# hellozhuo/svnet

Hardware: AMD Instinct MI355X
Metric: point-clouds/sec fwd+bwd, sv_dgcnn_cls B=32 N=1024 k=20 (higher is better)
Workload: dtype f32 (ternary bit-planes in the binarized layers); 1 GPU; sv_dgcnn_cls --binary fwd+loss+bwd, B=32 per GPU, N=1024, k=20; global_batch=32, parallelism=dp1, collective=none (1 rank), rccl_world=1, launch=hipGraph replay, binlinear=i8_mfma (>= 1024 rows) + xnor (head)

## Files before the change

include/svnet_hip.h:

```cpp
#ifndef SVNET_HIP_H
#define SVNET_HIP_H

#include <stddef.h>
#include <stdint.h>

#ifdef __cplusplus
extern "C" {
#endif

#define SVNET_OK 0
#define SVNET_E_ARG (-1)
#define SVNET_E_UNSUPPORTED (-2)
#define SVNET_E_WORKSPACE (-3)
#define SVNET_E_LAUNCH (-4)

#define SVNET_RED_SLICES 16
#define SVNET_SLICED_LEN(L) ((SVNET_RED_SLICES + 1) * (L) + 2)
int svnet_slices_sum_f32(float* buf, int64_t L, void* stream);
int svnet_slices_sum_f64(double* buf, int64_t L, void* stream);

#define SVNET_ABI_VERSION 417
int svnet_version(void);
const char* svnet_last_error(void);

typedef struct svnet_gate_fwd_job {
    const float* gin; const double* gin_f64; float* gin_out; float in_scale; const float* W0; const float* W2;
    int64_t B, Cin, H, Ov; float* h; float* gate;
    const float* rows; int64_t R;
} svnet_gate_fwd_job;
typedef struct svnet_gate_bwd_job {
    const float* dgate; const float* gate; const float* h; const float* gin; float in_scale; const float* W0; const float* W2;
    int64_t B, Cin, H, Ov; float out_scale; float* dgin; float* dW0; float* dW2;
} svnet_gate_bwd_job;

size_t svnet_knn_workspace_bytes(int64_t B, int64_t N, int64_t C);
int svnet_knn_f32(const float* x, int64_t B, int64_t N, int64_t C, int64_t sb, int64_t sn, int64_t sc,
                  int xx_mode, int k, int64_t* idx_out, void* workspace, size_t workspace_bytes, void* stream);
int svnet_knn_sv_f32(const float* s, int64_t Cs, const float* v, int64_t Cv3, int64_t B, int64_t N, int k, int64_t* idx_out,
                     void* workspace, size_t workspace_bytes, void* stream);

int svnet_knn_table_fusable(int64_t B, int64_t N, int64_t C);
int svnet_knn_from_table_f32(const void* workspace, size_t workspace_bytes, int64_t B, int64_t N, int64_t C, int k, int64_t* idx_out,
                             void* stream);
int svnet_edgeblock_apply_knn_f32(const int32_t* n_max, const int32_t* n_min, const float* mv, const float* mvn, const float* coef,
                                  const float* gate, int64_t P, int64_t N, int64_t Os, int64_t Ov, float slope, float* s_out, float* v_out,
                                  float* s_cat, int64_t s_ld, float* v_cat, int64_t v_ld, void* knn_workspace, size_t knn_workspace_bytes,
                                  void* stream);
int svnet_xyzblock_apply_knn_f32(const float* y_max, const float* y_min, const float* mv, const float* mvn, const float* coef,
                                 const float* gate, int64_t P, int64_t N, int64_t Os, int64_t Ov, float slope, float* s_out, float* v_out,
                                 float* s_cat, int64_t s_ld, float* v_cat, int64_t v_ld, void* knn_workspace, size_t knn_workspace_bytes,
                                 void* stream);

int svnet_edge_xyz_f32(const float* x, const int64_t* idx, int64_t B, int64_t N, int64_t k, int64_t m, int mode,
                       float* out, void* stream);

int svnet_edge_diffcat_fwd_f32(const float* table, const int64_t* idx, int idx_is_global, int64_t B, int64_t N,
                               int64_t k, int64_t G, int64_t F, float* out, void* stream);
int svnet_edge_diffcat_bwd_f32(const float* d_out, const int64_t* idx, int idx_is_global, int64_t B, int64_t N,
                               int64_t k, int64_t G, int64_t F, float* d_table, void* stream);

typedef struct svnet_gemm_desc {
    int64_t M, N, K;
    const float* A; int64_t a_rs, a_cs;
    const float* a_scale;
    const uint64_t* a_sign; const uint64_t* a_nz;
    const float* B; int64_t b_rs, b_cs;
    int b_exact;
    float* C; int64_t ldc, c_cs;
    float alpha;
    const float* col_scale;
    const float* bias;
    const uint64_t* mask;
    float* col_sum;
    int split_k;
    int accumulate;
    uint32_t tern_tile_mask;
    void* workspace;
    size_t workspace_bytes;
} svnet_gemm_desc;
size_t svnet_gemm_workspace_bytes(int64_t N, int64_t K);
int svnet_gemm_f32(const svnet_gemm_desc* desc, void* stream);

int svnet_binweight_prepare_f32(const float* W, const float* scale, int64_t O, int64_t K, uint64_t* w_sign,
                                uint64_t* w_nz, float* w_b, float* w_eff, void* stream);
int svnet_binlinear_fwd_f32(const float* x, int64_t ldx, const float* beta, const uint64_t* w_sign,
                            const uint64_t* w_nz, const float* scale, const float* bias, int64_t M, int64_t K,
                            int64_t O, float* y, uint64_t* x_sign, uint64_t* x_nz, uint64_t* x_ste, void* stream);
size_t svnet_binweight_i8_bytes(int64_t O, int64_t K);
int svnet_binweight_pack_i8(const float* W, int64_t O, int64_t K, int8_t* w_i8, void* stream);
int svnet_binlinear_i8_fwd_f32(const float* x, int64_t ldx, const float* beta, const int8_t* w_i8, const float* scale,
                               const float* bias, int64_t M, int64_t K, int64_t O, float* y, uint64_t* x_sign, uint64_t* x_nz,
                               uint64_t* x_ste, double* col_sums, void* stream);
int svnet_binlinear_i8_cloud_fwd_f32(const float* x, int64_t ldx, const float* beta, const int8_t* w_i8, const float* scale,
                                     const float* bias, int64_t M, int64_t K, int64_t O, float* y, uint64_t* x_sign, uint64_t* x_nz,
                                     uint64_t* x_ste, double* col_sums, const float* cloud_n, int64_t rows_per_cloud, void* stream);
int svnet_binweight_grad_f32(const float* GX, const float* W, const float* scale, int64_t O, int64_t K,
                             float* dW, float* dscale, int accumulate, int gx_sliced, float* sum_buf, int64_t sum_len, void* stream);

typedef struct svnet_edgeblock_desc {
    int64_t B, N, k;
    int Cs, Cv, Os, Ov;
    const float* s; const float* v; const int64_t* idx;
    const float* zz; const float* ut;
    const uint64_t* w_sign; const uint64_t* w_nz; const float* beta_perm;
    int32_t* n_max; int32_t* n_min; uint8_t* slot_max; uint8_t* slot_min;
    float* mv; float* mvn;
    int64_t* stat_n; double* stat_v; double* gate_sum;
    int16_t* n16; uint64_t* planes;
    const uint32_t* w_dense;
} svnet_edgeblock_desc;
int svnet_edgeblock_prepare_f32(const float* W, const float* beta, int64_t Os, int64_t Cs, int64_t Cv, uint64_t* w_sign,
                                uint64_t* w_nz, float* beta_perm , void* stream);
int svnet_edgeblock_prepare_vec_f32(const float* W2, const float* scale2, const float* Wz, const float* scalez, int64_t Ov,
                                    int64_t Cv, float* wv, float* scv, void* stream);
int svnet_edgeblock_fwd_f32(const svnet_edgeblock_desc* desc, void* stream);
int svnet_edgeblock_coeffs_f32(const int64_t* stat_n, const double* stat_v, int64_t E, int64_t Os, int64_t Ov,
                               const float* scale1, const float* gamma1, const float* beta1, float* running_mean1,
                               float* running_var1, const float* gamma2, const float* beta2, float* running_mean2,
                               float* running_var2, int training, float eps, float momentum, float* coef,
                               int64_t* num_batches_tracked1, int64_t* num_batches_tracked2 ,
                               const svnet_gate_fwd_job* gate_job , void* stream);
int svnet_edgeblock_apply_f32(const int32_t* n_max, const int32_t* n_min, const float* mv, const float* mvn,
                              const float* coef, const float* gate, int64_t P, int64_t N, int64_t Os, int64_t Ov,
                              float slope, float* s_out, float* v_out, float* s_cat, int64_t s_ld, float* v_cat, int64_t v_ld,
                              void* stream);

typedef struct svnet_block_tail_desc {
    const void* stat1; const double* stat_v; int64_t E, Os, Ov;
    const float* scale1;
    const float* gamma1; const float* beta1; float* running_mean1; float* running_var1;
    const float* gamma2; const float* beta2; float* running_mean2; float* running_var2;
    int training; float eps, momentum;
    float* coef; int64_t* num_batches_tracked1; int64_t* num_batches_tracked2;
    svnet_gate_fwd_job gate;
    const void* hi; const void* lo; const float* mv; const float* mvn;
    int64_t P, N; float slope;
    float* s_out; float* v_out; float* s_cat; int64_t s_ld; float* v_cat; int64_t v_ld;
    void* knn_workspace; size_t knn_workspace_bytes;
} svnet_block_tail_desc;
int svnet_block_tail_supported(int64_t P, int64_t N, int64_t Os, int64_t Ov, int with_knn_table);
int svnet_edgeblock_tail_f32(const svnet_block_tail_desc* desc, void* stream);
int svnet_xyzblock_tail_f32(const svnet_block_tail_desc* desc, void* stream);

#define SVNET_DBETA_SLICES 64
typedef struct svnet_edgeblock_bwd_desc {
    int64_t B, N, k;
    int Cs, Cv, Os, Ov;
    const float* v; const int64_t* idx; const float* zz; const float* ut;
    const int16_t* n16; const uint64_t* planes;
    const uint16_t* w1bt;
    const float* scale1;
    const uint8_t* slot_max; const uint8_t* slot_min;
    const float* coef;
    const float* gate;
    const float* gy;
    const float* bcoef;
    const float* gv;
    const float* gconst;
    float* dn_out; uint32_t* x_sign32; uint32_t* x_nz32;
    float* msg;
    float* ub_tab; float* ge_tab;
    float* ds_acc; float* dv_acc; float* dvc; float* dzc; float* dbeta_perm;
    int64_t* debug;
    int parts;
} svnet_edgeblock_bwd_desc;
int svnet_edgeblock_wbt_bf16(const uint64_t* w_sign, const uint64_t* w_nz, int64_t Os, int64_t Cs, int64_t Cv, uint16_t* wbt,
                             uint32_t* w_dense, void* stream);
int svnet_edgeblock_bwd_prelude_f32(const float* gs, const float* gv, const int32_t* n_max, const int32_t* n_min,
                                    const float* mv, const float* mvn, const float* coef, const float* scale1,
                                    const float* gate, int64_t P, int64_t N, int64_t Os, int64_t Ov, float slope,
                                    float* gy, float* red, float* redv, float* dgate,
                                    const float* gs2, int64_t gs2_ld, const float* gv2, int64_t gv2_ld, float* gv_sum, void* stream);
int svnet_edgeblock_bwd_coeffs_f32(const float* red, const float* redv, const float* coef, const float* gamma1,
                                   const float* gamma2, int64_t E, int64_t Os, int64_t Ov, int training, const float* scale1,
                                   float* bcoef, float* dgamma1, float* dbeta1, float* dgamma2, float* dbeta2,
                                   const svnet_gate_bwd_job* gate_job , void* stream);
int svnet_edgeblock_bwd_f32(const svnet_edgeblock_bwd_desc* desc, void* stream);
int svnet_knn_reverse_i32(const int64_t* idx, int64_t B, int64_t N, int64_t k, int32_t* rev_range, int32_t* rev_edge,
                          int32_t* rev_src, int64_t chunk, int32_t* ovf_items, int32_t* ovf_count, void* stream);
int64_t svnet_edgeblock_msg_stride(int64_t Cs, int64_t Cv, int64_t Ov);
int svnet_edgeblock_bwd_gather_f32(const float* msg, const int32_t* rev_range, const int32_t* rev_edge, const int32_t* rev_src,
                                   const float* ut, const float* ub_tab, const float* ge_tab, const float* coef, const float* bcoef,
                                   int64_t Os, const float* dvc, const float* dzc, int64_t P ,
                                   int64_t N , int64_t Cs, int64_t Cv,
                                   int64_t Ov, float* acat,
                                   int64_t acat_ld ,
                                   float* ds_acc, float* dv_acc, const float* dbeta_perm, float* dbeta1,
                                   int64_t chunk, const int32_t* ovf_items, const int32_t* ovf_count , void* stream);
int svnet_edgeblock_bwd_params_f32(const float* GXp, const float* GXc, const float* W1, const float* scale1, const float* W2,
                                   const float* scale2, const float* Wz, const float* scalez, int64_t Os, int64_t Ov,
                                   int64_t Cs, int64_t Cv, float* dW1, float* dscale1, float* dW2, float* dscale2, float* dWz,
                                   float* dscalez, void* stream);

typedef struct svnet_xyzblock_desc {
    int64_t B, N, k;
    int Os, Ov;
    const float* x; const int64_t* idx;
    const float* w0; const float* wz; const float* w1; const float* w2;
    float* y_max; float* y_min; uint8_t* slot_max; uint8_t* slot_min;
    float* mv; float* mvn;
    double* stat_y; double* stat_v; double* gate_sum;
    int64_t nc;
} svnet_xyzblock_desc;
int svnet_xyzblock_fwd_f32(const svnet_xyzblock_desc* desc, void* stream);
int svnet_xyzblock_coeffs_f32(const double* stat_y, const double* stat_v, int64_t E, int64_t Os, int64_t Ov,
                              const float* gamma1, const float* beta1, float* running_mean1, float* running_var1,
                              const float* gamma2, const float* beta2, float* running_mean2, float* running_var2,
                              int training, float eps, float momentum, float* coef, int64_t* num_batches_tracked1,
                              int64_t* num_batches_tracked2, const svnet_gate_fwd_job* gate_job , void* stream);
int svnet_xyzblock_apply_f32(const float* y_max, const float* y_min, const float* mv, const float* mvn, const float* coef,
                             const float* gate, int64_t P, int64_t N, int64_t Os, int64_t Ov, float slope, float* s_out,
                             float* v_out, float* s_cat, int64_t s_ld, float* v_cat, int64_t v_ld ,
                             void* stream);
int svnet_xyzblock_bwd_prelude_f32(const float* gs, const float* gv, const float* y_max, const float* y_min, const float* mv,
                                   const float* mvn, const float* coef, const float* gate, int64_t P, int64_t N, int64_t Os,
                                   int64_t Ov, float slope, float* gy, float* red, float* redv, float* dgate, const float* gs2,
                                   int64_t gs2_ld, const float* gv2, int64_t gv2_ld, float* gv_sum ,
                                   void* stream);
typedef struct svnet_xyzblock_bwd_desc {
    int64_t B, N, k;
    int Os, Ov;
    const float* x; const int64_t* idx;
    const float* w0; const float* wz; const float* w1; const float* w2;
    const uint8_t* slot_max; const uint8_t* slot_min;
    const float* coef; const float* bcoef; const float* gate; const float* gy; const float* gv; const float* gconst;
    float* gw;
    int64_t nc;
} svnet_xyzblock_bwd_desc;
int svnet_xyzblock_bwd_f32(const svnet_xyzblock_bwd_desc* desc, void* stream);

int svnet_edgeblock_wgrad_f32(const int16_t* n16, const uint8_t* slot_max, const uint8_t* slot_min, const float* gy,
                              const float* chc, const uint64_t* x_sign, const uint64_t* x_nz, int64_t E, int64_t k, int64_t Os,
                              float* GX, uint32_t q_tile_mask, void* stream);

int svnet_v2s_fwd_f32(const float* v, const float* w_eff, int64_t M, int64_t C, int64_t J, float* s, float* z_out,
                      void* stream);
int svnet_v2s_bwd_f32(const float* v, const float* w_eff, const float* ds, const float* dz_in, int64_t M, int64_t C,
                      int64_t J, float* dv, float* GX, void* stream);
int svnet_v2s_cat_fwd_f32(const float* v, const float* w_eff, const float* pre, int64_t pre_cols, int64_t M, int64_t C, int64_t J,
                          float* out, int64_t out_ld, void* stream);
int svnet_v2s_cat_sum_supported(int64_t M, int64_t C, int64_t pre_cols, int64_t rows_per_cloud);
int svnet_v2s_cat_sum_fwd_f32(const float* v, const float* w_eff, const float* pre, int64_t pre_cols, int64_t M, int64_t C, int64_t multi,
                              float* out, int64_t out_ld, double* pre_sum, int64_t rows_per_cloud, void* stream);
int svnet_v2s_bwd_ld_f32(const float* v, const float* w_eff, const float* ds, int64_t ds_ld, const float* dz_in, int64_t M, int64_t C,
                         int64_t J, float* dv, float* GX, void* stream);
int svnet_vproject_fwd_f32(const float* v, const float* z, int64_t M, int64_t C, int64_t J, float* s, void* stream);
int svnet_vproject_bwd_f32(const float* v, const float* z, const float* ds, int64_t M, int64_t C, int64_t J, float* dv,
                           float* dz, void* stream);

int svnet_colstats_f64(const float* x, int64_t M, int64_t C, int kind, double* sums, void* stream);
int svnet_vlinear_stats_f32(const float* v, int64_t P, int64_t K, const float* w_b, const float* col_scale, int64_t O, float* y,
                            double* sums, void* stream);
int svnet_bn_finalize_f32(double* sums, int64_t M, int64_t C, float eps, float momentum, float* mean,
                          float* invstd, float* running_mean, float* running_var, int64_t* num_batches_tracked,
                          void* stream);
int svnet_bn_eval_stats_f32(const float* running_mean, const float* running_var, int64_t C, float eps, float* mean,
                            float* invstd, void* stream);
int svnet_bn_act_fwd_f32(const float* x, const float* mean, const float* invstd, const float* gamma,
                         const float* beta, int64_t M, int64_t C, int act, float slope, float* y, void* stream);
int svnet_bn_act_bwd_reduce_f32(const float* g, const float* x, const float* mean, const float* invstd,
                                const float* gamma, const float* beta, int64_t M, int64_t C, int act, float slope,
                                float* red, void* stream);
int svnet_bn_act_bwd_apply_f32(const float* g, const float* x, const float* mean, const float* invstd,
                               const float* gamma, const float* beta, float* red, int64_t M, int64_t C, int act,
                               float slope, int train_stats, float* dx, void* stream);

int svnet_vbn_fwd_f32(const float* v, const float* mean, const float* invstd, const float* gamma, const float* beta,
                      const float* gate, int64_t rows_per_batch, int64_t M, int64_t C, float* out, void* stream);
int svnet_vbn_fwd_stats_f32(const float* v, const double* sums, float eps, float momentum, float* mean, float* invstd,
                            float* running_mean, float* running_var, int64_t* num_batches_tracked, const float* gamma,
                            const float* beta, const float* gate, int64_t rows_per_batch, int64_t M, int64_t C, float* out,
                            void* stream);
int svnet_vbn_bwd_reduce_f32(const float* g, const float* v, const float* mean, const float* invstd,
                             const float* gamma, const float* beta, const float* gate, int64_t rows_per_batch,
                             int64_t M, int64_t C, float* red, float* dgate, void* stream);
int svnet_vbn_bwd_apply_f32(const float* g, const float* v, const float* mean, const float* invstd,
                            const float* gamma, const float* beta, const float* gate, float* red,
                            int64_t rows_per_batch, int64_t M, int64_t C, int train_stats, float* dv, void* stream);

size_t svnet_pool_workspace_bytes(int64_t outer, int64_t R, int64_t inner, int mode);
int svnet_pool_fwd_f32(const float* x, int64_t outer, int64_t R, int64_t inner, int mode, float* out, int64_t out_ld,
                       int32_t* argmax, void* workspace, size_t workspace_bytes, void* stream);
int svnet_pool_maxmean_fwd_f32(const float* x, int64_t outer, int64_t R, int64_t inner, float* out_max, float* out_mean,
                               int64_t out_ld, int32_t* argmax, void* workspace, size_t workspace_bytes, void* stream);
int svnet_bn_pool_fwd_f32(const float* y, const float* mean, const float* invstd, const float* gamma, const float* beta,
                          int64_t outer, int64_t R, int64_t inner, int act, float slope, float* out_max, float* out_mean,
                          int64_t out_ld, int32_t* argmax, void* workspace, size_t workspace_bytes,
                          int workspace_zeroed ,
                          void* stream);
int svnet_bn_pool_bwd_f32(const float* gmax, const float* gmean, int64_t g_ld, const int32_t* argmax, const float* y,
                          const float* mean, const float* invstd, const float* gamma, const float* beta, int64_t outer, int64_t R,
                          int64_t inner, int act, float slope, int train_stats, float* red, float* dy, void* stream);
int svnet_pool_bwd_f32(const float* g, const int32_t* argmax, int64_t outer, int64_t R, int64_t inner, int mode,
                       float* dx, void* stream);
size_t svnet_vtail_workspace_bytes(int64_t B, int64_t N, int64_t C);
int svnet_vtail_fwd_f32(const float* v, const double* sums, float eps, float momentum, float* mean, float* invstd,
                        float* running_mean, float* running_var, long long* nbt, const float* gamma, const float* beta,
                        const float* gate, const float* w_eff, int64_t B, int64_t N, int64_t C, float* out_max, float* out_mean,
                        int64_t out_ld, int32_t* argmax, void* workspace, size_t workspace_bytes,
                        int workspace_zeroed , void* stream);
int svnet_vtail_bwd_f32(const float* v, const float* mean, const float* invstd, const float* gamma, const float* beta,
                        const float* gate, const float* w_eff, const float* gmax, const float* gmean, int64_t g_ld,
                        const int32_t* argmax, int64_t B, int64_t N, int64_t C, float* red, float* dgate, float* GX, float* g5,
                        void* stream);
int svnet_vtail_bwd_apply_f32(const float* v, const float* mean, const float* invstd, const float* gamma, const float* beta,
                              const float* gate, const float* w_eff, const float* gmax, const float* gmean, int64_t g_ld,
                              const int32_t* argmax, int64_t B, int64_t N, int64_t C, float* red, int train_stats, float* dv, void* stream);
int svnet_pool_mean_bwd_add_f32(const float* gmean, const float* add, int64_t add_ld, int64_t outer, int64_t R, int64_t inner,
                                float* dx, void* stream);
int svnet_pool_maxmean_bwd_f32(const float* gmax, const float* gmean, int64_t g_ld, const int32_t* argmax, int64_t outer, int64_t R,
                               int64_t inner, float* dx, void* stream);

int svnet_act_fwd_f32(const float* x, int64_t n, int kind, float* y, void* stream);
int svnet_act_bwd_f32(const float* g, const float* y, int64_t n, int kind, float* dx, void* stream);

int svnet_gate_mlp_fwd_f32(const float* gin, const double* gin_f64, float* gin_out, float in_scale, const float* W0,
                           const float* W2, int64_t B, int64_t Cin, int64_t H, int64_t Ov, float* h, float* gate,
                           const float* rows , int64_t R , void* stream);
int svnet_gate_mlp_bwd_f32(const float* dgate, const float* gate, const float* h, const float* gin, float in_scale,
                           const float* W0, const float* W2, int64_t B, int64_t Cin, int64_t H, int64_t Ov, float out_scale,
                           float* dgin, float* dW0, float* dW2, void* stream);

typedef struct svnet_binhead_desc {
    int64_t M, K, O;
    const float* W;
    const uint64_t* w_sign;
    const uint64_t* w_nz;
    int64_t wld;
    const float* w_b;
    const float* scale;
    const float* gamma;
    const float* bn_beta;
    float* running_mean;
    float* running_var;
    long long* nbt;
    int training;
    float eps, momentum;
    int act;
    float slope;
    const uint64_t* x_sign;
    const uint64_t* x_nz;
    const uint64_t* x_ste;
    const uint64_t* xc_sign;
    const uint64_t* xc_nz;
    float* y;
    float* mean;
    float* invstd;
    float* out;
    const float* g;
    float* dnT;
    float* dW;
    float* dscale;
    float* dgamma;
    float* dbn_beta;
    float* dx;
    float* dbeta_in;
} svnet_binhead_desc;
int svnet_binhead_pack_f32(const float* x, const float* beta, int64_t M, int64_t K, uint64_t* x_sign, uint64_t* x_nz,
                           uint64_t* x_ste, uint64_t* xc_sign, uint64_t* xc_nz, uint64_t* xc_ste, void* stream);
int svnet_binhead_fwd_f32(const svnet_binhead_desc* d, void* stream);
int svnet_binhead_bwd_f32(const svnet_binhead_desc* d, void* stream);
int svnet_fplinear_small_bwd_f32(const float* g, const float* x, const float* W, int64_t M, int64_t K, int64_t O, float* dx,
                                 float* dW, float* db, void* stream);

int svnet_smooth_ce_f32(const float* logits, const int64_t* target, int64_t R, int64_t C, float eps, float* loss,
                        float* dlogits, float* workspace, int64_t workspace_floats, void* stream);

int svnet_adam_step_f32(float* p, const float* g, float* m, float* v, int64_t n, float lr, float beta1, float beta2, float eps,
                        float weight_decay, int64_t step, void* stream);
int svnet_sgd_step_f32(float* p, const float* g, float* buf, int64_t n, float lr, float momentum, float weight_decay,
                       int first_step, void* stream);
int svnet_adam_step_dev_f32(float* p, const float* g, float* m, float* v, int64_t n, const float* hyper, void* stream);
int svnet_sgd_step_dev_f32(float* p, const float* g, float* buf, int64_t n, const float* hyper, void* stream);

int svnet_stamp_u64(uint64_t* slot, void* stream);

#ifdef __cplusplus
}
#endif
#endif
```

svnet_amd/_lib.py:

```python
import ctypes
import os
import subprocess

_HERE = os.path.dirname(os.path.abspath(__file__))
LIB_PATH = os.environ.get("SVNET_DIAG_LIB") or os.path.join(_HERE, "libsvnet_hip.so")
_lib = None
ABI_VERSION = 417

c_p = ctypes.c_void_p
c_i64 = ctypes.c_int64
c_int = ctypes.c_int
c_f = ctypes.c_float
c_sz = ctypes.c_size_t


class GemmDesc(ctypes.Structure):
    _fields_ = [
        ("M", c_i64), ("N", c_i64), ("K", c_i64),
        ("A", c_p), ("a_rs", c_i64), ("a_cs", c_i64),
        ("a_scale", c_p),
        ("a_sign", c_p), ("a_nz", c_p),
        ("B", c_p), ("b_rs", c_i64), ("b_cs", c_i64),
        ("b_exact", c_int),
        ("C", c_p), ("ldc", c_i64), ("c_cs", c_i64),
        ("alpha", c_f),
        ("col_scale", c_p),
        ("bias", c_p),
        ("mask", c_p),
        ("col_sum", c_p),
        ("split_k", c_int),
        ("accumulate", c_int),
        ("tern_tile_mask", ctypes.c_uint32),
        ("workspace", c_p),
        ("workspace_bytes", ctypes.c_size_t),
    ]


class GateFwdJob(ctypes.Structure):
    _fields_ = [("gin", c_p), ("gin_f64", c_p), ("gin_out", c_p), ("in_scale", c_f), ("W0", c_p), ("W2", c_p),
                ("B", c_i64), ("Cin", c_i64), ("H", c_i64), ("Ov", c_i64), ("h", c_p), ("gate", c_p), ("rows", c_p), ("R", c_i64)]


class BlockTailDesc(ctypes.Structure):
    _fields_ = [("stat1", c_p), ("stat_v", c_p), ("E", c_i64), ("Os", c_i64), ("Ov", c_i64), ("scale1", c_p),
                ("gamma1", c_p), ("beta1", c_p), ("running_mean1", c_p), ("running_var1", c_p),
                ("gamma2", c_p), ("beta2", c_p), ("running_mean2", c_p), ("running_var2", c_p),
                ("training", c_int), ("eps", c_f), ("momentum", c_f),
                ("coef", c_p), ("num_batches_tracked1", c_p), ("num_batches_tracked2", c_p),
                ("gate", GateFwdJob),
                ("hi", c_p), ("lo", c_p), ("mv", c_p), ("mvn", c_p), ("P", c_i64), ("N", c_i64), ("slope", c_f),
                ("s_out", c_p), ("v_out", c_p), ("s_cat", c_p), ("s_ld", c_i64), ("v_cat", c_p), ("v_ld", c_i64),
                ("knn_workspace", c_p), ("knn_workspace_bytes", c_sz)]


class GateBwdJob(ctypes.Structure):
    _fields_ = [("dgate", c_p), ("gate", c_p), ("h", c_p), ("gin", c_p), ("in_scale", c_f), ("W0", c_p), ("W2", c_p),
                ("B", c_i64), ("Cin", c_i64), ("H", c_i64), ("Ov", c_i64), ("out_scale", c_f), ("dgin", c_p), ("dW0", c_p), ("dW2", c_p)]


class EdgeBlockDesc(ctypes.Structure):
    _fields_ = [
        ("B", c_i64), ("N", c_i64), ("k", c_i64),
        ("Cs", c_int), ("Cv", c_int), ("Os", c_int), ("Ov", c_int),
        ("s", c_p), ("v", c_p), ("idx", c_p),
        ("zz", c_p), ("ut", c_p),
        ("w_sign", c_p), ("w_nz", c_p), ("beta_perm", c_p),
        ("n_max", c_p), ("n_min", c_p), ("slot_max", c_p), ("slot_min", c_p),
        ("mv", c_p), ("mvn", c_p),
        ("stat_n", c_p), ("stat_v", c_p), ("gate_sum", c_p),
        ("n16", c_p), ("planes", c_p),
        ("w_dense", c_p),
    ]


class EdgeBlockBwdDesc(ctypes.Structure):
    _fields_ = [
        ("B", c_i64), ("N", c_i64), ("k", c_i64),
        ("Cs", c_int), ("Cv", c_int), ("Os", c_int), ("Ov", c_int),
        ("v", c_p), ("idx", c_p), ("zz", c_p), ("ut", c_p),
        ("n16", c_p), ("planes", c_p),
        ("w1bt", c_p),
        ("scale1", c_p),
        ("slot_max", c_p), ("slot_min", c_p),
        ("coef", c_p), ("gate", c_p), ("gy", c_p), ("bcoef", c_p), ("gv", c_p), ("gconst", c_p),
        ("dn_out", c_p), ("x_sign32", c_p), ("x_nz32", c_p),
        ("msg", c_p),
        ("ub_tab", c_p), ("ge_tab", c_p),
        ("ds_acc", c_p), ("dv_acc", c_p), ("dvc", c_p), ("dzc", c_p), ("dbeta_perm", c_p),
        ("debug", c_p),
        ("parts", c_int),
    ]


class XyzBlockDesc(ctypes.Structure):
    _fields_ = [
        ("B", c_i64), ("N", c_i64), ("k", c_i64),
        ("Os", c_int), ("Ov", c_int),
        ("x", c_p), ("idx", c_p),
        ("w0", c_p), ("wz", c_p), ("w1", c_p), ("w2", c_p),
        ("y_max", c_p), ("y_min", c_p), ("slot_max", c_p), ("slot_min", c_p),
        ("mv", c_p), ("mvn", c_p),
        ("stat_y", c_p), ("stat_v", c_p), ("gate_sum", c_p),
        ("nc", c_i64),
    ]


class XyzBlockBwdDesc(ctypes.Structure):
    _fields_ = [
        ("B", c_i64), ("N", c_i64), ("k", c_i64),
        ("Os", c_int), ("Ov", c_int),
        ("x", c_p), ("idx", c_p),
        ("w0", c_p), ("wz", c_p), ("w1", c_p), ("w2", c_p),
        ("slot_max", c_p), ("slot_min", c_p),
        ("coef", c_p), ("bcoef", c_p), ("gate", c_p), ("gy", c_p), ("gv", c_p), ("gconst", c_p),
        ("gw", c_p),
        ("nc", c_i64),
    ]


class BinHeadDesc(ctypes.Structure):
    _fields_ = [
        ("M", c_i64), ("K", c_i64), ("O", c_i64),
        ("W", c_p), ("w_sign", c_p), ("w_nz", c_p), ("wld", c_i64), ("w_b", c_p),
        ("scale", c_p), ("gamma", c_p), ("bn_beta", c_p),
        ("running_mean", c_p), ("running_var", c_p), ("nbt", c_p),
        ("training", c_int), ("eps", c_f), ("momentum", c_f), ("act", c_int), ("slope", c_f),
        ("x_sign", c_p), ("x_nz", c_p), ("x_ste", c_p), ("xc_sign", c_p), ("xc_nz", c_p),
        ("y", c_p), ("mean", c_p), ("invstd", c_p), ("out", c_p),
        ("g", c_p), ("dnT", c_p), ("dW", c_p), ("dscale", c_p), ("dgamma", c_p), ("dbn_beta", c_p),
        ("dx", c_p), ("dbeta_in", c_p),
    ]


SIGNATURES = {
    "svnet_version": (c_int, []),
    "svnet_stamp_u64": (c_int, [c_p, c_p]),
    "svnet_slices_sum_f32": (c_int, [c_p, c_i64, c_p]),
    "svnet_slices_sum_f64": (c_int, [c_p, c_i64, c_p]),
    "svnet_last_error": (ctypes.c_char_p, []),
    "svnet_knn_workspace_bytes": (c_sz, [c_i64, c_i64, c_i64]),
    "svnet_knn_f32": (c_int, [c_p, c_i64, c_i64, c_i64, c_i64, c_i64, c_i64, c_int, c_int, c_p, c_p, c_sz, c_p]),
    "svnet_knn_sv_f32": (c_int, [c_p, c_i64, c_p, c_i64, c_i64, c_i64, c_int, c_p, c_p, c_sz, c_p]),
    "svnet_knn_table_fusable": (c_int, [c_i64, c_i64, c_i64]),
    "svnet_block_tail_supported": (c_int, [c_i64, c_i64, c_i64, c_i64, c_int]),
    "svnet_edgeblock_tail_f32": (c_int, [c_p, c_p]),
    "svnet_xyzblock_tail_f32": (c_int, [c_p, c_p]),
    "svnet_knn_from_table_f32": (c_int, [c_p, c_sz, c_i64, c_i64, c_i64, c_int, c_p, c_p]),
    "svnet_edge_xyz_f32": (c_int, [c_p, c_p, c_i64, c_i64, c_i64, c_i64, c_int, c_p, c_p]),
    "svnet_edge_diffcat_fwd_f32": (c_int, [c_p, c_p, c_int, c_i64, c_i64, c_i64, c_i64, c_i64, c_p, c_p]),
    "svnet_edge_diffcat_bwd_f32": (c_int, [c_p, c_p, c_int, c_i64, c_i64, c_i64, c_i64, c_i64, c_p, c_p]),
    "svnet_gemm_workspace_bytes": (ctypes.c_size_t, [c_i64, c_i64]),
    "svnet_gemm_f32": (c_int, [ctypes.POINTER(GemmDesc), c_p]),
    "svnet_binweight_prepare_f32": (c_int, [c_p, c_p, c_i64, c_i64, c_p, c_p, c_p, c_p, c_p]),
    "svnet_binlinear_fwd_f32": (c_int, [c_p, c_i64, c_p, c_p, c_p, c_p, c_p, c_i64, c_i64, c_i64, c_p, c_p, c_p, c_p, c_p]),
    "svnet_binweight_grad_f32": (c_int, [c_p, c_p, c_p, c_i64, c_i64, c_p, c_p, c_int, c_int, c_p, c_i64, c_p]),
    "svnet_edgeblock_prepare_vec_f32": (c_int, [c_p, c_p, c_p, c_p, c_i64, c_i64, c_p, c_p, c_p]),
    "svnet_knn_reverse_i32": (c_int, [c_p, c_i64, c_i64, c_i64, c_p, c_p, c_p, c_i64, c_p, c_p, c_p]),
    "svnet_edgeblock_msg_stride": (c_i64, [c_i64, c_i64, c_i64]),
    "svnet_edgeblock_bwd_gather_f32": (c_int, [c_p] * 9 + [c_i64] + [c_p, c_p] + [c_i64] * 5 + [c_p, c_i64, c_p, c_p, c_p, c_p, c_i64, c_p, c_p, c_p]),
    "svnet_edgeblock_bwd_params_f32": (c_int, [c_p] * 8 + [c_i64] * 4 + [c_p] * 6 + [c_p]),
    "svnet_edgeblock_prepare_f32": (c_int, [c_p, c_p, c_i64, c_i64, c_i64, c_p, c_p, c_p, c_p]),
    "svnet_edgeblock_fwd_f32": (c_int, [ctypes.POINTER(EdgeBlockDesc), c_p]),
    "svnet_edgeblock_coeffs_f32": (c_int, [c_p, c_p, c_i64, c_i64, c_i64, c_p, c_p, c_p, c_p, c_p, c_p, c_p, c_p, c_p, c_int, c_f, c_f, c_p, c_p, c_p, c_p, c_p]),
    "svnet_edgeblock_apply_f32": (c_int, [c_p, c_p, c_p, c_p, c_p, c_p, c_i64, c_i64, c_i64, c_i64, c_f, c_p, c_p, c_p, c_i64, c_p, c_i64, c_p]),
    "svnet_edgeblock_apply_knn_f32": (c_int, [c_p, c_p, c_p, c_p, c_p, c_p, c_i64, c_i64, c_i64, c_i64, c_f, c_p, c_p, c_p, c_i64, c_p, c_i64, c_p, c_sz, c_p]),
    "svnet_edgeblock_wbt_bf16": (c_int, [c_p, c_p, c_i64, c_i64, c_i64, c_p, c_p, c_p]),
    "svnet_edgeblock_bwd_prelude_f32": (c_int, [c_p] * 9 + [c_i64, c_i64, c_i64, c_i64, c_f, c_p, c_p, c_p, c_p, c_p, c_i64, c_p, c_i64, c_p, c_p]),
    "svnet_edgeblock_bwd_coeffs_f32": (c_int, [c_p, c_p, c_p, c_p, c_p, c_i64, c_i64, c_i64, c_int, c_p, c_p, c_p, c_p, c_p, c_p, c_p, c_p]),
    "svnet_edgeblock_bwd_f32": (c_int, [ctypes.POINTER(EdgeBlockBwdDesc), c_p]),
    "svnet_edgeblock_wgrad_f32": (c_int, [c_p, c_p, c_p, c_p, c_p, c_p, c_p, c_i64, c_i64, c_i64, c_p, ctypes.c_uint32, c_p]),
    "svnet_xyzblock_fwd_f32": (c_int, [ctypes.POINTER(XyzBlockDesc), c_p]),
    "svnet_xyzblock_coeffs_f32": (c_int, [c_p, c_p, c_i64, c_i64, c_i64, c_p, c_p, c_p, c_p, c_p, c_p, c_p, c_p, c_int, c_f, c_f, c_p, c_p, c_p, c_p, c_p]),
    "svnet_xyzblock_apply_f32": (c_int, [c_p, c_p, c_p, c_p, c_p, c_p, c_i64, c_i64, c_i64, c_i64, c_f, c_p, c_p, c_p, c_i64, c_p, c_i64, c_p]),
    "svnet_xyzblock_apply_knn_f32": (c_int, [c_p, c_p, c_p, c_p, c_p, c_p, c_i64, c_i64, c_i64, c_i64, c_f, c_p, c_p, c_p, c_i64, c_p, c_i64, c_p, c_sz, c_p]),
    "svnet_xyzblock_bwd_prelude_f32": (c_int, [c_p] * 8 + [c_i64, c_i64, c_i64, c_i64, c_f, c_p, c_p, c_p, c_p, c_p, c_i64, c_p, c_i64, c_p, c_p]),
    "svnet_xyzblock_bwd_f32": (c_int, [ctypes.POINTER(XyzBlockBwdDesc), c_p]),
    "svnet_binweight_i8_bytes": (c_sz, [c_i64, c_i64]),
    "svnet_binweight_pack_i8": (c_int, [c_p, c_i64, c_i64, c_p, c_p]),
    "svnet_binlinear_i8_fwd_f32": (c_int, [c_p, c_i64, c_p, c_p, c_p, c_p, c_i64, c_i64, c_i64, c_p, c_p, c_p, c_p, c_p, c_p]),
    "svnet_binlinear_i8_cloud_fwd_f32": (c_int, [c_p, c_i64, c_p, c_p, c_p, c_p, c_i64, c_i64, c_i64, c_p, c_p, c_p, c_p, c_p, c_p, c_i64, c_p]),
    "svnet_v2s_fwd_f32": (c_int, [c_p, c_p, c_i64, c_i64, c_i64, c_p, c_p, c_p]),
    "svnet_v2s_bwd_f32": (c_int, [c_p, c_p, c_p, c_p, c_i64, c_i64, c_i64, c_p, c_p, c_p]),
    "svnet_v2s_cat_fwd_f32": (c_int, [c_p, c_p, c_p, c_i64, c_i64, c_i64, c_i64, c_p, c_i64, c_p]),
    "svnet_v2s_cat_sum_supported": (c_int, [c_i64, c_i64, c_i64, c_i64]),
    "svnet_v2s_cat_sum_fwd_f32": (c_int, [c_p, c_p, c_p, c_i64, c_i64, c_i64, c_i64, c_p, c_i64, c_p, c_i64, c_p]),
    "svnet_v2s_bwd_ld_f32": (c_int, [c_p, c_p, c_p, c_i64, c_p, c_i64, c_i64, c_i64, c_p, c_p, c_p]),
    "svnet_vproject_fwd_f32": (c_int, [c_p, c_p, c_i64, c_i64, c_i64, c_p, c_p]),
    "svnet_vproject_bwd_f32": (c_int, [c_p, c_p, c_p, c_i64, c_i64, c_i64, c_p, c_p, c_p]),
    "svnet_colstats_f64": (c_int, [c_p, c_i64, c_i64, c_int, c_p, c_p]),
    "svnet_bn_finalize_f32": (c_int, [c_p, c_i64, c_i64, c_f, c_f, c_p, c_p, c_p, c_p, c_p, c_p]),
    "svnet_bn_eval_stats_f32": (c_int, [c_p, c_p, c_i64, c_f, c_p, c_p, c_p]),
    "svnet_bn_act_fwd_f32": (c_int, [c_p, c_p, c_p, c_p, c_p, c_i64, c_i64, c_int, c_f, c_p, c_p]),
    "svnet_bn_act_bwd_reduce_f32": (c_int, [c_p, c_p, c_p, c_p, c_p, c_p, c_i64, c_i64, c_int, c_f, c_p, c_p]),
    "svnet_bn_act_bwd_apply_f32": (c_int, [c_p, c_p, c_p, c_p, c_p, c_p, c_p, c_i64, c_i64, c_int, c_f, c_int, c_p, c_p]),
    "svnet_vbn_fwd_f32": (c_int, [c_p, c_p, c_p, c_p, c_p, c_p, c_i64, c_i64, c_i64, c_p, c_p]),
    "svnet_vbn_fwd_stats_f32": (c_int, [c_p, c_p, c_f, c_f, c_p, c_p, c_p, c_p, c_p, c_p, c_p, c_p, c_i64, c_i64, c_i64, c_p, c_p]),
    "svnet_vbn_bwd_reduce_f32": (c_int, [c_p, c_p, c_p, c_p, c_p, c_p, c_p, c_i64, c_i64, c_i64, c_p, c_p, c_p]),
    "svnet_vbn_bwd_apply_f32": (c_int, [c_p, c_p, c_p, c_p, c_p, c_p, c_p, c_p, c_i64, c_i64, c_i64, c_int, c_p, c_p]),
    "svnet_pool_workspace_bytes": (c_sz, [c_i64, c_i64, c_i64, c_int]),
    "svnet_pool_fwd_f32": (c_int, [c_p, c_i64, c_i64, c_i64, c_int, c_p, c_i64, c_p, c_p, c_sz, c_p]),
    "svnet_pool_maxmean_fwd_f32": (c_int, [c_p, c_i64, c_i64, c_i64, c_p, c_p, c_i64, c_p, c_p, c_sz, c_p]),
    "svnet_bn_pool_fwd_f32": (c_int, [c_p] * 5 + [c_i64] * 3 + [c_int, c_f, c_p, c_p, c_i64, c_p, c_p, c_sz, c_int, c_p]),
    "svnet_bn_pool_bwd_f32": (c_int, [c_p, c_p, c_i64] + [c_p] * 6 + [c_i64] * 3 + [c_int, c_f, c_int, c_p, c_p, c_p]),
    "svnet_pool_bwd_f32": (c_int, [c_p, c_p, c_i64, c_i64, c_i64, c_int, c_p, c_p]),
    "svnet_pool_mean_bwd_add_f32": (c_int, [c_p, c_p, c_i64, c_i64, c_i64, c_i64, c_p, c_p]),
    "svnet_pool_maxmean_bwd_f32": (c_int, [c_p, c_p, c_i64, c_p, c_i64, c_i64, c_i64, c_p, c_p]),
    "svnet_vtail_workspace_bytes": (c_sz, [c_i64, c_i64, c_i64]),
    "svnet_vtail_fwd_f32": (c_int, [c_p, c_p, c_f, c_f] + [c_p] * 9 + [c_i64] * 3 + [c_p, c_p, c_i64, c_p, c_p, c_sz, c_int, c_p]),
    "svnet_vtail_bwd_f32": (c_int, [c_p] * 9 + [c_i64, c_p] + [c_i64] * 3 + [c_p] * 5),
    "svnet_vtail_bwd_apply_f32": (c_int, [c_p] * 9 + [c_i64, c_p] + [c_i64] * 3 + [c_p, c_int, c_p, c_p]),
    "svnet_act_fwd_f32": (c_int, [c_p, c_i64, c_int, c_p, c_p]),
    "svnet_act_bwd_f32": (c_int, [c_p, c_p, c_i64, c_int, c_p, c_p]),
    "svnet_vlinear_stats_f32": (c_int, [c_p, c_i64, c_i64, c_p, c_p, c_i64, c_p, c_p, c_p]),
    "svnet_gate_mlp_fwd_f32": (c_int, [c_p, c_p, c_p, c_f, c_p, c_p, c_i64, c_i64, c_i64, c_i64, c_p, c_p, c_p, c_i64, c_p]),
    "svnet_gate_mlp_bwd_f32": (c_int, [c_p, c_p, c_p, c_p, c_f, c_p, c_p, c_i64, c_i64, c_i64, c_i64, c_f, c_p, c_p, c_p, c_p]),
    "svnet_adam_step_f32": (c_int, [c_p, c_p, c_p, c_p, c_i64, c_f, c_f, c_f, c_f, c_f, c_i64, c_p]),
    "svnet_sgd_step_f32": (c_int, [c_p, c_p, c_p, c_i64, c_f, c_f, c_f, c_int, c_p]),
    "svnet_adam_step_dev_f32": (c_int, [c_p, c_p, c_p, c_p, c_i64, c_p, c_p]),
    "svnet_sgd_step_dev_f32": (c_int, [c_p, c_p, c_p, c_i64, c_p, c_p]),
    "svnet_smooth_ce_f32": (c_int, [c_p, c_p, c_i64, c_i64, c_f, c_p, c_p, c_p, c_i64, c_p]),
    "svnet_binhead_pack_f32": (c_int, [c_p, c_p, c_i64, c_i64, c_p, c_p, c_p, c_p, c_p, c_p, c_p]),
    "svnet_binhead_fwd_f32": (c_int, [ctypes.POINTER(BinHeadDesc), c_p]),
    "svnet_binhead_bwd_f32": (c_int, [ctypes.POINTER(BinHeadDesc), c_p]),
    "svnet_fplinear_small_bwd_f32": (c_int, [c_p, c_p, c_p, c_i64, c_i64, c_i64, c_p, c_p, c_p, c_p]),
}


class SvnetHipError(RuntimeError):
    pass


def build(force=False, verbose=False):
    cmd = ["make", "-C", os.path.join(_HERE, "csrc"), "-j8"] + (["-B"] if force else [])
    res = subprocess.run(cmd, stdout=subprocess.PIPE, stderr=subprocess.STDOUT, text=True)
    if verbose or res.returncode != 0:
        print(res.stdout)
    if res.returncode != 0:
        raise SvnetHipError("building libsvnet_hip.so failed")
    return LIB_PATH


def lib():
    global _lib
    if _lib is None:
        if not os.path.exists(LIB_PATH):
            raise SvnetHipError(
                "%s is missing: run `python -c 'import __graft_entry__ as g; g.build()'` (or make -C svnet_amd/csrc). "
                "svnet_amd has no CPU fallback." % LIB_PATH)
        handle = ctypes.CDLL(LIB_PATH)
        for name, (res, args) in SIGNATURES.items():
            fn = getattr(handle, name)
            fn.restype = res
            fn.argtypes = args
        if handle.svnet_version() != ABI_VERSION:
            raise SvnetHipError("%s was built for ABI %d, this binding speaks %d (include/svnet_hip.h SVNET_ABI_VERSION): rebuild it"
                                % (LIB_PATH, handle.svnet_version(), ABI_VERSION))
        _lib = handle
    return _lib


def check(code, what):
    if code != 0:
        msg = lib().svnet_last_error()
        raise SvnetHipError("%s failed (%d): %s" % (what, code, msg.decode() if msg else "?"))


class KernelTimer:

    def __init__(self, name, select=None):
        self.name, self.select, self.pairs = name, select, []

    def elapsed_ms(self):
        return [a.elapsed_time(b) for a, b in self.pairs]


TIMERS = []


class StepClock:

    def __init__(self, device, select=None, slots=4096):
        import torch
        self.buf = torch.zeros(slots, dtype=torch.int64, device=device)
        self.names, self.select = [], select

    def mark(self, name):
        import torch
        if self.select is not None and not self.select(name):
            return
        i = len(self.names)
        if i >= self.buf.numel():
            return
        st = torch.cuda.current_stream(self.buf.device)
        self.names.append((name, st.cuda_stream))
        lib().svnet_stamp_u64(ctypes.c_void_p(self.buf.data_ptr() + 8 * i), ctypes.c_void_p(st.cuda_stream))

    def read(self):
        t = self.buf[:len(self.names)].cpu().tolist()
        t0 = min(t) if t else 0
        return sorted(((x - t0) / 100.0, n, s) for x, (n, s) in zip(t, self.names))


CLOCK = None


def call(name, *args):
    fn = getattr(lib(), name)
    if CLOCK is not None:
        CLOCK.mark(name)
    hit = [t for t in TIMERS if t.name == name and (t.select is None or t.select(args))] if TIMERS else None
    if hit:
        import torch
        a, b = torch.cuda.Event(enable_timing=True), torch.cuda.Event(enable_timing=True)
        st = torch.cuda.current_stream()
        a.record(st)
        rc = fn(*args)
        b.record(st)
        for t in hit:
            t.pairs.append((a, b))
    else:
        rc = fn(*args)
    if rc != 0:
        msg = lib().svnet_last_error()
        raise SvnetHipError("%s failed (%d): %s" % (name, rc, msg.decode() if msg else "?"))
```

svnet_amd/_ops.py:

```python
import ctypes

import torch

from . import _lib, config
from ._lib import BinHeadDesc, GemmDesc, call

BN_EPS = 1e-5
RED_SLICES = 16
BN_MOMENTUM = 0.1

TAP = None



def _p(t):
    return None if t is None else ctypes.c_void_p(t.data_ptr())


def _stream():
    return ctypes.c_void_p(torch.cuda.current_stream().cuda_stream)


def _hip(*tensors):
    for t in tensors:
# ... 643 lines not shown
    return out


class BinLinearCloud(torch.autograd.Function):

    @staticmethod
    def forward(ctx, x_cloud, x_point, W, beta, scale, training=True, cloud_at=0):
        global _FUSED_COLSUMS
        _hip(x_cloud, x_point, W, beta, scale)
        ctx.training = bool(training)
        B, N, Kp = x_point.shape
        Kc = x_cloud.shape[-1]
        k0 = int(cloud_at)
        xp = _f32c(x_point).reshape(B * N, Kp)
        xc = _f32c(x_cloud).reshape(B, Kc)
        W_in, Wc = W, _f32c(W).reshape(W.shape[0], -1)
        O, K = Wc.shape
        if K != Kc + Kp or not 0 <= k0 <= Kp:
            raise ValueError("BinLinearCloud: weight has %d columns, inputs %d + %d (cloud block at %d)" % (K, Kc, Kp, k0))
        M = B * N
        dev = xp.device
        need_grad = any(ctx.needs_input_grad)
        sc, bt = _f32c(scale).view(-1), _f32c(beta).view(-1)
        bt_c = bt[k0:k0 + Kc]
        bt_p = bt[Kc:] if k0 == 0 else torch.cat([bt[:k0], bt[k0 + Kc:]])
        pk_c = _binweight_cols(W_in, scale, [(k0, k0 + Kc)])
        pk_p = _binweight_cols(W_in, scale, [(0, k0), (k0 + Kc, K)], i8=True)
        keep = need_grad or TAP is not None
        pl_c = [torch.empty(((B + 63) // 64, Kc), dtype=torch.int64, device=dev) for _ in range(3)] if keep else [None] * 3
        pl_p = [torch.empty(((M + 63) // 64, Kp), dtype=torch.int64, device=dev) for _ in range(3)] if keep else [None] * 3
        ones = torch.ones((O,), dtype=torch.float32, device=dev)
        n_cloud = torch.empty((B, O), dtype=torch.float32, device=dev)
        call("svnet_binlinear_fwd_f32", _p(xc), Kc, _p(bt_c), _p(pk_c["w_sign"]), _p(pk_c["w_nz"]), _p(ones), None, B, Kc, O, _p(n_cloud),
             _p(pl_c[0]), _p(pl_c[1]), _p(pl_c[2]), _stream())
        y = torch.empty((M, O), dtype=torch.float32, device=dev)
        sums = _zeros((_sliced_len(2 * O),), torch.float64, dev) if (training and config.FUSE_BN_STATS and K <= 46340) else None
        call("svnet_binlinear_i8_cloud_fwd_f32", _p(xp), Kp, _p(bt_p), _p(pk_p["w_i8"]), _p(sc), None, M, Kp, O, _p(y),
             _p(pl_p[0]), _p(pl_p[1]), _p(pl_p[2]), _p(sums), _p(n_cloud), N, _stream())
        _FUSED_COLSUMS = (y, y._version, sums) if sums is not None else None
        if TAP is not None:
            full = [torch.cat([b[:, :k0], a, b[:, k0:]], dim=1).contiguous() for a, b in zip(_cloud_planes_as_rows(pl_c, B, N, Kc), pl_p)]
            TAP["signs"].append(("rows", M, K, full))
        if need_grad:
            ctx.save_for_backward(Wc, sc, pk_c["w_b"], pk_p["w_b"], *pl_c, *pl_p)
        ctx.meta = (B, N, Kc, Kp, O, x_cloud.shape, x_point.shape, beta.shape, scale.shape, W_in.shape, k0)
        return y.view(B, N, O)

    @staticmethod
    def backward(ctx, g):
        Wc, sc, wb_c, wb_p, cs, cz, cq, ps, pz, pq = ctx.saved_tensors
        B, N, Kc, Kp, O, cshape, pshape, bshape, sshape, wshape, k0 = ctx.meta
        K, M = Kc + Kp, B * N
        dev = g.device
        g2 = _f32c(g).reshape(M, O)
        gc = pool_raw(g2, B, N, O, 1)[0]
        gc = gc * float(N)
        need_w = ctx.needs_input_grad[2] or ctx.needs_input_grad[4]
        dxc = dxp = dbeta = dW = dsc = None
        dbuf_c = _zeros((_sliced_len(Kc),), torch.float32, dev)
        dbuf_p = _zeros((_sliced_len(Kp),), torch.float32, dev)
        if ctx.training:
            dxp = torch.empty((M, Kp), dtype=torch.float32, device=dev)
            gemm(M, Kp, O, A=g2, a_rs=O, a_cs=1, a_scale=sc, B=wb_p, b_rs=Kp, b_cs=1, b_exact=True, C=dxp, ldc=Kp, mask=pq, col_sum=dbuf_p)
            dxc = torch.empty((B, Kc), dtype=torch.float32, device=dev)
            gemm(B, Kc, O, A=gc, a_rs=O, a_cs=1, a_scale=sc, B=wb_c, b_rs=Kc, b_cs=1, b_exact=True, C=dxc, ldc=Kc, mask=cq, col_sum=dbuf_c)
            call("svnet_slices_sum_f32", _p(dbuf_p), Kp, _stream())
            call("svnet_slices_sum_f32", _p(dbuf_c), Kc, _stream())
        else:
            dxp = torch.zeros((M, Kp), dtype=torch.float32, device=dev)
            dxc = torch.zeros((B, Kc), dtype=torch.float32, device=dev)
        dbeta = torch.cat([dbuf_p[:k0], dbuf_c[:Kc], dbuf_p[k0:Kp]]).view(bshape)
        if need_w:
            if k0 == 0:
                GX = _zeros((O, K), torch.float32, dev)
                gemm(Kc, O, B, a_planes=(cs, cz), B=gc, b_rs=O, b_cs=1, C=GX, ldc=1, c_cs=K, accumulate=True)
                gemm(Kp, O, M, a_planes=(ps, pz), B=g2, b_rs=O, b_cs=1, C=GX[:, Kc:], ldc=1, c_cs=K, accumulate=True)
            else:
                GXc, GXp = _zeros((O, Kc), torch.float32, dev), _zeros((O, Kp), torch.float32, dev)
                gemm(Kc, O, B, a_planes=(cs, cz), B=gc, b_rs=O, b_cs=1, C=GXc, ldc=1, c_cs=Kc, accumulate=True)
                gemm(Kp, O, M, a_planes=(ps, pz), B=g2, b_rs=O, b_cs=1, C=GXp, ldc=1, c_cs=Kp, accumulate=True)
                GX = torch.cat([GXp[:, :k0], GXc, GXp[:, k0:]], dim=1)
            dW, dsc = _binweight_grad(GX, Wc, sc, O, K, ctx.training)
            dW, dsc = dW.view(wshape), dsc.view(sshape)
        return dxc.view(cshape), dxp.view(pshape), dW, dbeta, dsc, None, None


class BinLinearBNAct(torch.autograd.Function):

    @staticmethod
    def supported(M, K, O):
        return 1 <= M <= 64 and K <= 3776 and O >= 1

    @staticmethod
    def forward(ctx, x, W, beta, scale, gamma, bn_beta, running_mean, running_var, training, act, slope, nbt=None, eps=BN_EPS,
                momentum=BN_MOMENTUM, want_grad=True):
        _hip(x, W, beta, scale, gamma, bn_beta)
        x2 = _f32c(x).reshape(-1, x.shape[-1])
        W_in, Wc = W, _f32c(W).reshape(W.shape[0], -1)
        M, K = x2.shape
        O = Wc.shape[0]
        KW = _words(K)
        dev = x.device
        need_grad = bool(want_grad) and any(ctx.needs_input_grad)
        if need_grad and not training:
            raise RuntimeError("svnet_amd: BinLinearBNAct has no eval-mode backward (use BinLinear + BNAct)")
        packed = _binweight(W_in, scale)
        sc, bt = _f32c(scale).view(-1), _f32c(beta).view(-1)
        keep = need_grad or TAP is not None
        rowp = torch.empty((3, M, KW), dtype=torch.int64, device=dev)
        colp = torch.empty((3, K), dtype=torch.int64, device=dev) if keep else None
        call("svnet_binhead_pack_f32", _p(x2), _p(bt), M, K, _p(rowp[0]), _p(rowp[1]), _p(rowp[2]),
             _p(colp[0]) if keep else None, _p(colp[1]) if keep else None, _p(colp[2]) if keep else None, _stream())
        y = torch.empty((M, O), dtype=torch.float32, device=dev)
        out = torch.empty((M, O), dtype=torch.float32, device=dev)
        stats = torch.empty((2, O), dtype=torch.float32, device=dev)
        d = BinHeadDesc()
        d.M, d.K, d.O = M, K, O
        d.w_sign, d.w_nz, d.wld = _p(packed["w_sign"]), _p(packed["w_nz"]), KW
        d.scale, d.gamma, d.bn_beta = _p(sc), _p(gamma), _p(bn_beta)
        d.running_mean, d.running_var, d.nbt = _p(running_mean), _p(running_var), _p(nbt)
        d.training, d.eps, d.momentum, d.act, d.slope = int(bool(training)), eps, momentum, int(act), slope
        d.x_sign, d.x_nz = _p(rowp[0]), _p(rowp[1])
        d.y, d.mean, d.invstd, d.out = _p(y), _p(stats[0]), _p(stats[1]), _p(out)
        call("svnet_binhead_fwd_f32", ctypes.byref(d), _stream())
        if TAP is not None:
            TAP["signs"].append(("rows", M, K, [colp[0].view(1, K), colp[1].view(1, K), colp[2].view(1, K)]))
            _tap_act(gamma, act, out)
        if need_grad:
            ctx.save_for_backward(Wc, sc, packed["w_b"], rowp, colp, y, stats, gamma, bn_beta)
        ctx.meta = (M, K, O, KW, x.shape, beta.shape, scale.shape, W_in.shape, int(act), slope)
        return out.view(x.shape[:-1] + (O,))

    @staticmethod
    def backward(ctx, g):
        Wc, sc, w_b, rowp, colp, y, stats, gamma, bn_beta = ctx.saved_tensors
        M, K, O, KW, xshape, bshape, sshape, wshape, act, slope = ctx.meta
        dev = g.device
        g2 = _f32c(g).reshape(M, O)
        need_x = ctx.needs_input_grad[0] or ctx.needs_input_grad[2]
        need_w = ctx.needs_input_grad[1]
        dnT = torch.empty((O, 64), dtype=torch.float32, device=dev)
        dW = torch.empty((O, K), dtype=torch.float32, device=dev) if need_w else None
        small = torch.empty((3, O), dtype=torch.float32, device=dev)
        dx = torch.empty((M, K), dtype=torch.float32, device=dev) if need_x else None
        dbeta = torch.empty((K,), dtype=torch.float32, device=dev) if need_x else None
        d = BinHeadDesc()
        d.M, d.K, d.O = M, K, O
        d.W, d.w_b, d.wld = _p(Wc), _p(w_b), KW
        d.scale, d.gamma, d.bn_beta = _p(sc), _p(gamma), _p(bn_beta)
        d.training, d.act, d.slope = 1, act, slope
        d.x_ste, d.xc_sign, d.xc_nz = _p(rowp[2]), _p(colp[0]), _p(colp[1])
        d.y, d.mean, d.invstd = _p(y), _p(stats[0]), _p(stats[1])
        d.g, d.dnT, d.dW = _p(g2), _p(dnT), _p(dW)
        d.dscale, d.dgamma, d.dbn_beta = _p(small[0]), _p(small[1]), _p(small[2])
        d.dx, d.dbeta_in = _p(dx), _p(dbeta)
        call("svnet_binhead_bwd_f32", ctypes.byref(d), _stream())
        return (dx.view(xshape) if dx is not None else None, dW.view(wshape) if dW is not None else None,
                dbeta.view(bshape) if dbeta is not None else None, small[0].view(sshape), small[1], small[2],
                None, None, None, None, None, None, None, None, None)



class V2S(torch.autograd.Function):

    @staticmethod
    def forward(ctx, v, W, scale, training=True):
        _hip(v, W, scale)
        ctx.training = bool(training)
        ctx.set_materialize_grads(False)
        v3 = _f32c(v).reshape(-1, 3, v.shape[-1])
        W_in, W = W, _f32c(W)
        M, _, C = v3.shape
        J = W.shape[0]
        if scale is not None:
            sc = _f32c(scale).view(-1)
            w_eff = _binweight(W_in, scale)["w_eff"]
        else:
            sc, w_eff = None, W
        s = torch.empty((M, C * J), dtype=torch.float32, device=v.device)
        z = torch.empty((M, 3, J), dtype=torch.float32, device=v.device)
        call("svnet_v2s_fwd_f32", _p(v3), _p(w_eff), M, C, J, _p(s), _p(z), _stream())
        ctx.save_for_backward(v3, W, w_eff, sc)
        ctx.vshape = v.shape
        ctx.sshape = None if scale is None else scale.shape
        lead = v.shape[:-2]
        return s.view(lead + (C * J,)), z.view(lead + (3, J))

    @staticmethod
    def backward(ctx, gs, gz):
        v3, W, w_eff, sc = ctx.saved_tensors
        M, _, C = v3.shape
        J = W.shape[0]
        L = _lib.lib()
        gs2 = torch.zeros((M, C * J), dtype=torch.float32, device=v3.device) if gs is None else _f32c(gs).reshape(M, C * J)
        gz2 = None if gz is None else _f32c(gz).reshape(M, 3, J)
        dv = torch.empty_like(v3)
        gxb = _zeros((_sliced_len(J * C),), torch.float32, v3.device)
        call("svnet_v2s_bwd_f32", _p(v3), _p(w_eff), _p(gs2), _p(gz2), M, C, J, _p(dv), _p(gxb), _stream())
        if sc is not None:
            dW, dsc = _binweight_grad(gxb, W, sc, J, C, ctx.training, gx_sliced=True)
            dsc = dsc.view(ctx.sshape)
        else:
            call("svnet_slices_sum_f32", _p(gxb), J * C, _stream())
            dW, dsc = gxb[:J * C].view(J, C), None
        return dv.view(ctx.vshape), dW, dsc, None


class V2SCat(torch.autograd.Function):

    @staticmethod
    def forward(ctx, s, v, W, scale, training=True, clouds=0, gate_W0=None, gate_W2=None):
        _hip(s, v, W, scale)
        ctx.training = bool(training)
        v3 = _f32c(v).reshape(-1, 3, v.shape[-1])
        M, _, C = v3.shape
        s2 = _f32c(s).reshape(M, s.shape[-1])
        Cs = s2.shape[1]
        W_in, W = W, _f32c(W)
        J = W.shape[0]
        if scale is not None:
            sc = _f32c(scale).view(-1)
            w_eff = _binweight(W_in, scale)["w_eff"]
        else:
            sc, w_eff = None, W
        out = torch.empty((M, Cs + C * J), dtype=torch.float32, device=v.device)
        ctx.meta = (M, C, J, Cs, s.shape, v.shape, None if scale is None else scale.shape)
        ctx.clouds = int(clouds)
        ctx.set_materialize_grads(False)
        cat = out.view(s.shape[:-1] + (Cs + C * J,))
        ctx.with_gate = False
        if clouds and gate_W0 is not None and _lib.lib().svnet_v2s_cat_sum_supported(M, C, Cs, M // clouds):
            rows = M // clouds
            s_sum = _zeros((clouds, Cs), torch.float64, v.device)
            call("svnet_v2s_cat_sum_fwd_f32", _p(v3), _p(w_eff), _p(s2), Cs, M, C, J, _p(out), Cs + C * J, _p(s_sum), rows, _stream())
            W0c, W2c = _f32c(gate_W0), _f32c(gate_W2)
            H, Ov = W0c.shape[0], W2c.shape[0]
            pooled = torch.empty((clouds, Cs), dtype=torch.float32, device=v.device)
            h = torch.empty((clouds, H), dtype=torch.float32, device=v.device)
            gate = torch.empty((clouds, Ov), dtype=torch.float32, device=v.device)
            call("svnet_gate_mlp_fwd_f32", None, _p(s_sum), _p(pooled), 1.0 / float(rows), _p(W0c), _p(W2c), clouds, Cs, H, Ov, _p(h), _p(gate),
                 None, 0, _stream())
            _tap_act(gate_W0, 2, h)
            ctx.save_for_backward(v3, W, w_eff, sc, pooled, W0c, W2c, h, gate)
            ctx.with_gate = True
            ctx.gate_in_scale = 1.0 / float(rows)
            return cat, gate
        call("svnet_v2s_cat_fwd_f32", _p(v3), _p(w_eff), _p(s2), Cs, M, C, J, _p(out), Cs + C * J, _stream())
        ctx.save_for_backward(v3, W, w_eff, sc)
        if clouds:
            s_mean, _ = pool_raw(s2, clouds, M // clouds, Cs, 1)
            if gate_W0 is not None:
                W0c, W2c = _f32c(gate_W0), _f32c(gate_W2)
                H, Ov = W0c.shape[0], W2c.shape[0]
                h = torch.empty((clouds, H), dtype=torch.float32, device=v.device)
                gate = torch.empty((clouds, Ov), dtype=torch.float32, device=v.device)
                call("svnet_gate_mlp_fwd_f32", _p(s_mean), None, None, 1.0, _p(W0c), _p(W2c), clouds, Cs, H, Ov, _p(h), _p(gate), None, 0, _stream())
                _tap_act(gate_W0, 2, h)
                ctx.save_for_backward(v3, W, w_eff, sc, s_mean, W0c, W2c, h, gate)
                ctx.with_gate = True
                ctx.gate_in_scale = 1.0
                return cat, gate
            return cat, s_mean
        return cat

    @staticmethod
    def backward(ctx, g, g_mean=None):
        dW0 = dW2 = None
        if ctx.with_gate:
            v3, W, w_eff, sc, pooled, W0g, W2g, hg, gateg = ctx.saved_tensors
            if g_mean is not None:
                Bc, Cin = pooled.shape
                H, Ov = W0g.shape[0], W2g.shape[0]
                zb = _zeros((H * Cin + Ov * H,), torch.float32, pooled.device)
                dW0, dW2 = zb[:H * Cin].view(H, Cin), zb[H * Cin:].view(Ov, H)
                dmean = torch.empty_like(pooled)
                call("svnet_gate_mlp_bwd_f32", _p(_f32c(g_mean)), _p(gateg), _p(hg), _p(pooled), ctx.gate_in_scale, _p(W0g), _p(W2g), Bc, Cin, H, Ov,
                     1.0, _p(dmean), _p(dW0), _p(dW2), _stream())
                g_mean = dmean
        else:
            v3, W, w_eff, sc = ctx.saved_tensors
        M, C, J, Cs, sshape, vshape, scshape = ctx.meta
        if g is None:
            g = torch.zeros((M, Cs + C * J), dtype=torch.float32, device=v3.device)
        g2 = _f32c(g).reshape(M, Cs + C * J)
        ds = None
        if ctx.needs_input_grad[0]:
            if g_mean is not None:
                ds = torch.empty((M, Cs), dtype=torch.float32, device=g2.device)
                call("svnet_pool_mean_bwd_add_f32", _p(_f32c(g_mean).reshape(ctx.clouds, Cs)), _p(g2), Cs + C * J, ctx.clouds, M // ctx.clouds, Cs,
                     _p(ds), _stream())
                ds = ds.reshape(sshape)
            else:
                ds = g2[:, :Cs].reshape(sshape)
        dv = torch.empty_like(v3)
        gxb = _zeros((_sliced_len(J * C),), torch.float32, v3.device)
        call("svnet_v2s_bwd_ld_f32", _p(v3), _p(w_eff), _p(g2[:, Cs:]), Cs + C * J, None, M, C, J, _p(dv), _p(gxb), _stream())
        if sc is not None:
            dW, dsc = _binweight_grad(gxb, W, sc, J, C, ctx.training, gx_sliced=True)
            dsc = dsc.view(scshape)
        else:
            call("svnet_slices_sum_f32", _p(gxb), J * C, _stream())
            dW, dsc = gxb[:J * C].view(J, C), None
        return ds, dv.view(vshape), dW, dsc, None, None, dW0, dW2


class VProject(torch.autograd.Function):

    @staticmethod
    def forward(ctx, v, z):
        _hip(v, z)
        v3 = _f32c(v).reshape(-1, 3, v.shape[-1])
        z3 = _f32c(z).reshape(-1, 3, z.shape[-1])
        M, _, C = v3.shape
        J = z3.shape[-1]
        s = torch.empty((M, C * J), dtype=torch.float32, device=v.device)
        call("svnet_vproject_fwd_f32", _p(v3), _p(z3), M, C, J, _p(s), _stream())
        ctx.save_for_backward(v3, z3)
        ctx.shapes = (v.shape, z.shape)
        return s.view(v.shape[:-2] + (C * J,))

    @staticmethod
    def backward(ctx, gs):
        v3, z3 = ctx.saved_tensors
        M, _, C = v3.shape
        J = z3.shape[-1]
        gs2 = _f32c(gs).reshape(M, C * J)
        dv, dz = torch.empty_like(v3), torch.empty_like(z3)
        call("svnet_vproject_bwd_f32", _p(v3), _p(z3), _p(gs2), M, C, J, _p(dv), _p(dz), _stream())
        return dv.view(ctx.shapes[0]), dz.view(ctx.shapes[1])



_FUSED_COLSUMS = None
_FUSED_VSTATS = None


def _batch_stats(x, M, C, kind, running_mean, running_var, training, momentum, eps, nbt=None):
    global _FUSED_COLSUMS
    L = _lib.lib()
    dev = x.device
    mean = torch.empty((C,), dtype=torch.float32, device=dev)
    invstd = torch.empty((C,), dtype=torch.float32, device=dev)
    if training:
        rec, _FUSED_COLSUMS = _FUSED_COLSUMS, None
        if (kind == 0 and rec is not None and rec[0].data_ptr() == x.data_ptr() and tuple(rec[0].shape) == (M, C)
                and rec[0]._version == rec[1] and x.is_contiguous()):
            sums = rec[2]
        else:
            sums = _zeros((_sliced_len(2 * C),), torch.float64, dev)
            call("svnet_colstats_f64", _p(x), M, C, kind, _p(sums), _stream())
        call("svnet_bn_finalize_f32", _p(sums), M, C, eps, momentum, _p(mean), _p(invstd), _p(running_mean), _p(running_var),
                                      _p(nbt), _stream())
    else:
        call("svnet_bn_eval_stats_f32", _p(running_mean), _p(running_var), C, eps, _p(mean), _p(invstd), _stream())
    return mean, invstd


def _tap_act(gamma, act, out):
    if TAP is not None and "acts" in TAP and act in (1, 2):
        TAP["acts"].append((gamma.data_ptr(), (out > 0).reshape(-1, out.shape[-1])))


class BNAct(torch.autograd.Function):

    @staticmethod
    def forward(ctx, x, gamma, beta, running_mean, running_var, training, act, slope, nbt=None, eps=BN_EPS, momentum=BN_MOMENTUM):
        _hip(x, gamma, beta)
        x2 = _f32c(x).reshape(-1, x.shape[-1])
        M, C = x2.shape
        mean, invstd = _batch_stats(x2, M, C, 0, running_mean, running_var, training, momentum, eps, nbt)
        y = torch.empty_like(x2)
        call("svnet_bn_act_fwd_f32", _p(x2), _p(mean), _p(invstd), _p(gamma), _p(beta), M, C, act, slope, _p(y), _stream())
        _tap_act(gamma, act, y)
        ctx.save_for_backward(x2, mean, invstd, gamma, beta)
        ctx.meta = (M, C, act, slope, bool(training), x.shape)
        return y.view(x.shape)

    @staticmethod
    def backward(ctx, g):
        x2, mean, invstd, gamma, beta = ctx.saved_tensors
        M, C, act, slope, training, xshape = ctx.meta
        L = _lib.lib()
        g2 = _f32c(g).reshape(M, C)
        red = _zeros((_sliced_len(2 * C),), torch.float32, g.device)
        call("svnet_bn_act_bwd_reduce_f32", _p(g2), _p(x2), _p(mean), _p(invstd), _p(gamma), _p(beta), M, C, act, slope, _p(red),
                                            _stream())
        dx = None
        if ctx.needs_input_grad[0]:
            dx = torch.empty_like(x2)
            call("svnet_bn_act_bwd_apply_f32", _p(g2), _p(x2), _p(mean), _p(invstd), _p(gamma), _p(beta), _p(red), M, C, act, slope,
                                               int(training), _p(dx), _stream())
            dx = dx.view(xshape)
        else:
            call("svnet_slices_sum_f32", _p(red), 2 * C, _stream())
        return dx, red[C:2 * C], red[:C], None, None, None, None, None, None, None, None


class VBN(torch.autograd.Function):

    @staticmethod
    def forward(ctx, v, gamma, beta, running_mean, running_var, gate, rows_per_batch, training, nbt=None, eps=BN_EPS, momentum=BN_MOMENTUM):
        _hip(v, gamma, beta, gate)
        v3 = _f32c(v).reshape(-1, 3, v.shape[-1])
        M, _, C = v3.shape
        gate2 = None if gate is None else _f32c(gate).reshape(-1, C)
        out = torch.empty_like(v3)
        global _FUSED_VSTATS
        rec, _FUSED_VSTATS = _FUSED_VSTATS, None
        if training and M > 0:
            if (rec is not None and rec[0].data_ptr() == v3.data_ptr() and rec[0].numel() == v3.numel() and rec[0]._version == rec[1]
                    and tuple(rec[0].shape) == (3 * M, C)):
                sums = rec[2]
            else:
                sums = _zeros((_sliced_len(2 * C),), torch.float64, v3.device)
                call("svnet_colstats_f64", _p(v3), M, C, 1, _p(sums), _stream())
            mean = torch.empty((C,), dtype=torch.float32, device=v3.device)
            invstd = torch.empty((C,), dtype=torch.float32, device=v3.device)
            call("svnet_vbn_fwd_stats_f32", _p(v3), _p(sums), eps, momentum, _p(mean), _p(invstd), _p(running_mean), _p(running_var), _p(nbt),
                 _p(gamma), _p(beta), _p(gate2), rows_per_batch, M, C, _p(out), _stream())
        else:
            mean, invstd = _batch_stats(v3, M, C, 1, running_mean, running_var, training, momentum, eps, nbt)
            call("svnet_vbn_fwd_f32", _p(v3), _p(mean), _p(invstd), _p(gamma), _p(beta), _p(gate2), rows_per_batch, M, C, _p(out),
                                               _stream())
        ctx.save_for_backward(v3, mean, invstd, gamma, beta, gate2)
        ctx.meta = (M, C, rows_per_batch, bool(training), v.shape, None if gate is None else gate.shape)
        return out.view(v.shape)

    @staticmethod
    def backward(ctx, g):
        v3, mean, invstd, gamma, beta, gate2 = ctx.saved_tensors
        M, C, rpb, training, vshape, gshape = ctx.meta
        L = _lib.lib()
        g3 = _f32c(g).reshape(M, 3, C)
        if gate2 is None:
            red, dgate = _zeros((_sliced_len(2 * C),), torch.float32, g.device), None
        else:
            red, dgate = _zeros_pool(g.device, ((_sliced_len(2 * C),), torch.float32), (tuple(gate2.shape), torch.float32))
        call("svnet_vbn_bwd_reduce_f32", _p(g3), _p(v3), _p(mean), _p(invstd), _p(gamma), _p(beta), _p(gate2), rpb, M, C, _p(red),
                                         _p(dgate), _stream())
        dv = None
        if ctx.needs_input_grad[0]:
            dv = torch.empty_like(v3)
            call("svnet_vbn_bwd_apply_f32", _p(g3), _p(v3), _p(mean), _p(invstd), _p(gamma), _p(beta), _p(gate2), _p(red), rpb, M, C,
                                            int(training), _p(dv), _stream())
            dv = dv.view(vshape)
        else:
            call("svnet_slices_sum_f32", _p(red), 2 * C, _stream())
        if dgate is not None:
            dgate = dgate.view(gshape)
        return dv, red[C:2 * C], red[:C], None, None, dgate, None, None, None, None, None



def pool_raw(x, outer, R, inner, mode, out=None):
    if out is None:
        out = torch.empty((outer, inner), dtype=torch.float32, device=x.device)
    arg = torch.empty((outer, inner), dtype=torch.int32, device=x.device) if mode == 0 else None
    nbytes = _lib.lib().svnet_pool_workspace_bytes(outer, R, inner, mode)
    ws = torch.empty((nbytes,), dtype=torch.uint8, device=x.device) if nbytes else None
    call("svnet_pool_fwd_f32", _p(x), outer, R, inner, mode, _p(out), out.stride(0), _p(arg), _p(ws), nbytes, _stream())
    return out, arg


def pool_maxmean_raw(x, outer, R, inner, out_max, out_mean):
    L = _lib.lib()
    nb0, nb1 = L.svnet_pool_workspace_bytes(outer, R, inner, 0), L.svnet_pool_workspace_bytes(outer, R, inner, 1)
    if R >= 256 and nb0 and nb1 and out_max.stride(0) == out_mean.stride(0):
        arg = torch.empty((outer, inner), dtype=torch.int32, device=x.device)
        ws = torch.empty((nb0 + nb1,), dtype=torch.uint8, device=x.device)
        call("svnet_pool_maxmean_fwd_f32", _p(x), outer, R, inner, _p(out_max), _p(out_mean), out_max.stride(0), _p(arg), _p(ws), nb0 + nb1,
             _stream())
        return arg
    _, arg = pool_raw(x, outer, R, inner, 0, out=out_max)
    pool_raw(x, outer, R, inner, 1, out=out_mean)
    return arg


class Pool(torch.autograd.Function):

    @staticmethod
    def forward(ctx, x, dim, mode):
        _hip(x)
        x = _f32c(x)
        dim = dim % x.dim()
        outer = 1
        for d in x.shape[:dim]:
            outer *= d
        R = x.shape[dim]
        inner = 1
        for d in x.shape[dim + 1:]:
            inner *= d
        out, arg = pool_raw(x, outer, R, inner, mode)
        if arg is not None:
            ctx.save_for_backward(arg)
            if TAP is not None:
                TAP["pools"].append(arg)
        ctx.meta = (outer, R, inner, mode, x.shape)
        return out.view(x.shape[:dim] + x.shape[dim + 1:])

    @staticmethod
    def backward(ctx, g):
        outer, R, inner, mode, xshape = ctx.meta
        arg = ctx.saved_tensors[0] if mode == 0 else None
        g2 = _f32c(g).reshape(outer, inner)
        dx = torch.empty(xshape, dtype=torch.float32, device=g.device)
        call("svnet_pool_bwd_f32", _p(g2), _p(arg), outer, R, inner, mode, _p(dx), _stream())
        return dx, None, None


class PoolMaxParts(torch.autograd.Function):

    @staticmethod
    def forward(ctx, a, b):
        _hip(a, b)
        a, b = _f32c(a), _f32c(b)
        B, N, Ca = a.shape
        Cb = b.shape[-1]
        out = torch.empty((B, Ca + Cb), dtype=torch.float32, device=a.device)
        _, arg_a = pool_raw(a, B, N, Ca, 0, out=out[:, :Ca])
        _, arg_b = pool_raw(b, B, N, Cb, 0, out=out[:, Ca:])
        ctx.save_for_backward(arg_a, arg_b)
        if TAP is not None:
            TAP["pools"].append(torch.cat([arg_a, arg_b], dim=1))
        ctx.meta = (B, N, Ca, Cb)
        return out

    @staticmethod
    def backward(ctx, g):
        B, N, Ca, Cb = ctx.meta
        arg_a, arg_b = ctx.saved_tensors
        g = _f32c(g)
        ga, gb = g[:, :Ca].contiguous(), g[:, Ca:].contiguous()
        da = torch.empty((B, N, Ca), dtype=torch.float32, device=g.device)
        db = torch.empty((B, N, Cb), dtype=torch.float32, device=g.device)
        call("svnet_pool_bwd_f32", _p(ga), _p(arg_a), B, N, Ca, 0, _p(da), _stream())
        call("svnet_pool_bwd_f32", _p(gb), _p(arg_b), B, N, Cb, 0, _p(db), _stream())
        return da, db


class PoolMaxMean(torch.autograd.Function):

    @staticmethod
    def forward(ctx, x, dim):
        _hip(x)
        x = _f32c(x)
        dim = dim % x.dim()
        outer = 1
        for d in x.shape[:dim]:
            outer *= d
        R = x.shape[dim]
        inner = 1
        for d in x.shape[dim + 1:]:
            inner *= d
        out = torch.empty((outer, 2 * inner), dtype=torch.float32, device=x.device)
        arg = pool_maxmean_raw(x, outer, R, inner, out[:, :inner], out[:, inner:])
        ctx.save_for_backward(arg)
        if TAP is not None:
            TAP["pools"].append(arg)
        ctx.meta = (outer, R, inner, x.shape)
        return out.view(x.shape[:dim] + (2 * inner,)) if x.dim() - dim == 2 else out

    @staticmethod
    def backward(ctx, g):
        outer, R, inner, xshape = ctx.meta
        (arg,) = ctx.saved_tensors
        g2 = _f32c(g).reshape(outer, 2 * inner)
        dx = torch.empty(xshape, dtype=torch.float32, device=g.device)
        call("svnet_pool_maxmean_bwd_f32", _p(g2), _p(g2[:, inner:]), 2 * inner, _p(arg), outer, R, inner, _p(dx), _stream())
        return dx, None


class GlobalMaxMeanPool(torch.autograd.Function):

    @staticmethod
    def forward(ctx, a, b):
        _hip(a, b)
        a, b = _f32c(a), _f32c(b)
        B, N, Ca = a.shape
        Cb = b.shape[-1]
        C = Ca + Cb
        out = torch.empty((B, 2 * C), dtype=torch.float32, device=a.device)
        main, side = torch.cuda.current_stream(a.device), _side_stream(a.device)
        side.wait_stream(main)
        with torch.cuda.stream(side):
            arg_b = pool_maxmean_raw(b, B, N, Cb, out[:, Ca:C], out[:, C + Ca:])
            arg_b.record_stream(main)
        arg_a = pool_maxmean_raw(a, B, N, Ca, out[:, :Ca], out[:, C:C + Ca])
        main.wait_stream(side)
        ctx.save_for_backward(arg_a, arg_b)
        if TAP is not None:
            TAP["pools"].append(torch.cat([arg_a, arg_b], dim=1))
        ctx.meta = (B, N, Ca, Cb)
        return out

    @staticmethod
    def backward(ctx, g):
        B, N, Ca, Cb = ctx.meta
        arg_a, arg_b = ctx.saved_tensors
        C = Ca + Cb
        g = _f32c(g)
        da = torch.empty((B, N, Ca), dtype=torch.float32, device=g.device)
        db = torch.empty((B, N, Cb), dtype=torch.float32, device=g.device)
        main, side = torch.cuda.current_stream(g.device), _side_stream(g.device)
        side.wait_stream(main)
        with torch.cuda.stream(side):
            call("svnet_pool_maxmean_bwd_f32", _p(g[:, Ca:]), _p(g[:, C + Ca:]), 2 * C, _p(arg_b), B, N, Cb, _p(db), _stream())
# ... 829 lines not shown
```

svnet_amd/config.py:

```python
import os

DEBUG_FINITE = os.environ.get("SVNET_DEBUG_FINITE", "0") not in ("", "0")

FUSE_EDGE_BLOCKS = True

TWO_STREAM_BLOCKS = True
TWO_STREAM_MIN_ROWS = 4096

GATHER_CHUNK = 128

DW_BESIDE = False

FUSE_BN_POOL = True

FUSE_VTAIL = True
FUSE_VTAIL_APPLY = True

FUSE_V2S_CAT = True

BINLINEAR_MFMA = True

FUSE_BN_STATS = True

SPLIT_BROADCAST = True

FUSE_HEAD = True
DEFER_WGRAD = True
VEC_EARLY = True
DEFER_ROWS_WGRAD = True
ROWS2_MIN_K = 64

MAIN_PRIORITY = 0
SIDE_PRIORITY = 0

FUSE_VBN_STATS = False

GATE_MEAN_INSIDE = True

EDGE_DENSE_WEIGHTS = True
KNN_TABLE_AHEAD = True
FUSE_BLOCK_TAIL = True
FUSE_CAT_MEAN = True
```

svnet_amd/csrc/binlinear_mfma.hip:

```cpp
#include "common.h"

namespace {

typedef __attribute__((ext_vector_type(4))) int i32x4;
typedef __attribute__((ext_vector_type(16))) int i32x16;

constexpr int BM = 128;
constexpr int KC = 128;
constexpr int LDA = KC + 16;

__global__ __launch_bounds__(256) void binweight_pack_i8_kernel(const float* __restrict__ W, int O, int K, int Kp, int8_t* __restrict__ out) {
    const int total = O * Kp;
    for (int e = blockIdx.x * blockDim.x + threadIdx.x; e < total; e += gridDim.x * blockDim.x) {
        const int o = e / Kp, p = e - o * Kp;
        const int c = p >> 7, pin = p & 127;
        const int k = c * KC + 32 * (pin & 3) + (pin >> 2);
        const float w = k < K ? W[(int64_t)o * K + k] : 0.f;
        out[e] = (int8_t)((w > 0.f) - (w < 0.f));
    }
}

template <int NTW>
__global__ __launch_bounds__(1024, 4) void binlinear_i8_fwd_kernel(const float* __restrict__ x, int64_t ldx, const float* __restrict__ beta,
                                                                   const int8_t* __restrict__ w8, const float* __restrict__ scale,
                                                                   const float* __restrict__ bias, int64_t M, int K, int O, int Kp,
                                                                   float* __restrict__ y, uint32_t* __restrict__ x_sign32,
                                                                   uint32_t* __restrict__ x_nz32, uint32_t* __restrict__ x_ste32,
                                                                   double* __restrict__ col_sums, const float* __restrict__ cloud_n,
                                                                   int64_t rows_per_cloud) {
    constexpr int OT = 128 * NTW;
    extern __shared__ __attribute__((aligned(16))) unsigned char bl_lds[];
    int8_t* At = reinterpret_cast<int8_t*>(bl_lds);
    int8_t* Bt = At + BM * LDA;
    uint64_t* pw = reinterpret_cast<uint64_t*>(Bt + OT * LDA);
    const int tid = threadIdx.x, lane = tid & 63;
    const int wave = __builtin_amdgcn_readfirstlane(tid >> 6);
    const int r = lane & 31, h = lane >> 5;
    const int wr = wave >> 2, wc = wave & 3;
    const int64_t m0 = (int64_t)blockIdx.x * BM;
    const int o0 = blockIdx.y * OT;
    const bool save = x_sign32 != nullptr && blockIdx.y == 0;

    i32x16 acc[NTW];
#pragma unroll
    for (int t = 0; t < NTW; ++t)
#pragma unroll
        for (int i = 0; i < 16; ++i) acc[t][i] = 0;

    const int nchunks = Kp / KC;
    float xa[4][4];
    const int64_t brow = min(m0 + 8 * wave, M - 1);
    const float* xbase = x + brow * ldx;
    uint32_t rowb[4];
#pragma unroll
    for (int rp = 0; rp < 4; ++rp) rowb[rp] = (uint32_t)(min(m0 + 8 * wave + h + 2 * rp, M - 1) - brow) * (uint32_t)ldx * 4u;
#define SVNET_BL_LOAD_A(K0)                                                                       \
    do {                                                                                          \
        uint32_t colb_[4];                                                                        \
        _Pragma("unroll") for (int j = 0; j < 4; ++j) colb_[j] = 4u * (uint32_t)min((K0) + 32 * j + r, K - 1); \
        _Pragma("unroll") for (int rp = 0; rp < 4; ++rp)                                          \
            _Pragma("unroll") for (int j = 0; j < 4; ++j) xa[rp][j] = ld_f32_sbase(xbase, rowb[rp] + colb_[j]); \
    } while (0)
    SVNET_BL_LOAD_A(0);
    for (int c = 0; c < nchunks; ++c) {
        const int k0 = c * KC;
        uint4 bstage[NTW];
#pragma unroll
        for (int u = 0; u < NTW; ++u) {
            const int e = tid + 1024 * u;
            const int n = e >> 3, pc = e & 7;
            const int o = min(o0 + n, O - 1);
            bstage[u] = *reinterpret_cast<const uint4*>(w8 + (int64_t)o * Kp + k0 + 16 * pc);
        }
        {
            float bt[4];
#pragma unroll
            for (int j = 0; j < 4; ++j) bt[j] = beta[min(k0 + 32 * j + r, K - 1)];
#pragma unroll
            for (int rp = 0; rp < 4; ++rp) {
                const int row = 8 * wave + 2 * rp + h;
                uint32_t pk = 0;
                uint64_t bs[4], bz[4], bq[4];
#pragma unroll
                for (int j = 0; j < 4; ++j) {
                    const bool in = (k0 + 32 * j + r) < K && (m0 + row) < M;
                    const float tv = in ? xa[rp][j] + bt[j] : 0.f;
                    const bool pos = tv > 0.f, neg = tv < 0.f;
                    pk |= (pos ? 0x01u : (neg ? 0xFFu : 0u)) << (8 * j);
                    if (save) {
                        bs[j] = __ballot(pos);
                        bz[j] = __ballot(pos || neg);
                        bq[j] = __ballot(in && fabsf(tv) <= 1.2f);
                    } else {
                        bs[j] = bz[j] = bq[j] = 0ull;
                    }
                }
                *reinterpret_cast<uint32_t*>(&At[row * LDA + 4 * r]) = pk;
                if (save && lane == 0) {
                    const int ra = 8 * wave + 2 * rp;
#pragma unroll
                    for (int hh = 0; hh < 2; ++hh) {
                        const int sh = 32 * hh;
                        pw[(0 * BM + ra + hh) * 2 + 0] = ((bs[0] >> sh) & 0xFFFFFFFFull) | (((bs[1] >> sh) & 0xFFFFFFFFull) << 32);
                        pw[(0 * BM + ra + hh) * 2 + 1] = ((bs[2] >> sh) & 0xFFFFFFFFull) | (((bs[3] >> sh) & 0xFFFFFFFFull) << 32);
                        pw[(1 * BM + ra + hh) * 2 + 0] = ((bz[0] >> sh) & 0xFFFFFFFFull) | (((bz[1] >> sh) & 0xFFFFFFFFull) << 32);
                        pw[(1 * BM + ra + hh) * 2 + 1] = ((bz[2] >> sh) & 0xFFFFFFFFull) | (((bz[3] >> sh) & 0xFFFFFFFFull) << 32);
                        pw[(2 * BM + ra + hh) * 2 + 0] = ((bq[0] >> sh) & 0xFFFFFFFFull) | (((bq[1] >> sh) & 0xFFFFFFFFull) << 32);
                        pw[(2 * BM + ra + hh) * 2 + 1] = ((bq[2] >> sh) & 0xFFFFFFFFull) | (((bq[3] >> sh) & 0xFFFFFFFFull) << 32);
                    }
                }
            }
        }
#pragma unroll
        for (int u = 0; u < NTW; ++u) {
            const int e = tid + 1024 * u;
            *reinterpret_cast<uint4*>(&Bt[(e >> 3) * LDA + 16 * (e & 7)]) = bstage[u];
        }
        __syncthreads();
        SVNET_BL_LOAD_A(min(k0 + KC, (nchunks - 1) * KC));
        __builtin_amdgcn_sched_barrier(0);
        if (save) {
            for (int item = wave; item < 24; item += 16) {
                const int plane = item >> 3, rb = (item >> 2) & 1, cg = item & 3;
                const uint64_t wrd = pw[(plane * BM + 64 * rb + lane) * 2 + (cg >> 1)];
                const uint32_t mine = (cg & 1) ? (uint32_t)(wrd >> 32) : (uint32_t)wrd;
                const uint32_t colword = svnet_bit_transpose32(mine, lane);
                const int k = k0 + 32 * cg + (lane & 31);
                const int64_t blk = (m0 >> 6) + rb;
                if (k < K && blk * 64 < M) {
                    uint32_t* dst = plane == 0 ? x_sign32 : (plane == 1 ? x_nz32 : x_ste32);
                    dst[(blk * K + k) * 2 + (lane >> 5)] = colword;
                }
            }
        }
#pragma unroll
        for (int s = 0; s < KC / 32; ++s) {
            const i32x4 af = *reinterpret_cast<const i32x4*>(&At[(32 * wr + r) * LDA + 32 * s + 16 * h]);
#pragma unroll
            for (int t = 0; t < NTW; ++t) {
                const i32x4 bf = *reinterpret_cast<const i32x4*>(&Bt[(32 * (NTW * wc + t) + r) * LDA + 32 * s + 16 * h]);
                acc[t] = __builtin_amdgcn_mfma_i32_32x32x32_i8(af, bf, acc[t], 0, 0, 0);
            }
        }
        __syncthreads();
    }
#undef SVNET_BL_LOAD_A
    if (cloud_n) {
#pragma unroll
        for (int t = 0; t < NTW; ++t) {
            const int o = min(o0 + 32 * (NTW * wc + t) + r, O - 1);
#pragma unroll
            for (int i = 0; i < 16; ++i) {
                const int64_t m = min(m0 + 32 * wr + (i & 3) + 8 * (i >> 2) + 4 * h, M - 1);
                acc[t][i] += (int)cloud_n[(m / rows_per_cloud) * O + o];
            }
        }
    }
#pragma unroll
    for (int t = 0; t < NTW; ++t) {
        const int o = o0 + 32 * (NTW * wc + t) + r;
        if (o < O) {
            const float sc = scale[o], bs = bias ? bias[o] : 0.f;
#pragma unroll
            for (int i = 0; i < 16; ++i) {
                const int64_t m = m0 + 32 * wr + (i & 3) + 8 * (i >> 2) + 4 * h;
                if (m < M) y[m * O + o] = (float)acc[t][i] * sc + bs;
            }
        }
    }
    if (col_sums) {
        long long* red = reinterpret_cast<long long*>(bl_lds);
        for (int i = tid; i < 2 * OT; i += 1024) red[i] = 0;
        __syncthreads();
#pragma unroll
        for (int t = 0; t < NTW; ++t) {
            int s1 = 0;
            long long s2 = 0;
#pragma unroll
            for (int i = 0; i < 16; ++i) {
                const int64_t m = m0 + 32 * wr + (i & 3) + 8 * (i >> 2) + 4 * h;
                const int c = m < M ? acc[t][i] : 0;
                s1 += c;
                s2 += (long long)(c * c);
            }
            atomicAdd(reinterpret_cast<unsigned long long*>(&red[32 * (NTW * wc + t) + r]), (unsigned long long)(long long)s1);
            atomicAdd(reinterpret_cast<unsigned long long*>(&red[OT + 32 * (NTW * wc + t) + r]), (unsigned long long)s2);
        }
        __syncthreads();
        const int o = o0 + tid;
        if (tid < OT && o < O) {
            const double sc = (double)scale[o], bs = bias ? (double)bias[o] : 0.0;
            const double S1 = (double)red[tid], S2 = (double)red[OT + tid];
            const double R = (double)min((int64_t)BM, M - m0);
            double* sl = svnet_slice_ptr(col_sums, 2 * O);
            svnet_slice_add(&sl[o], sc * S1 + R * bs);
            svnet_slice_add(&sl[O + o], sc * sc * S2 + 2.0 * sc * bs * S1 + R * bs * bs);
        }
    }
}

}

extern "C" size_t svnet_binweight_i8_bytes(int64_t O, int64_t K) { return (O > 0 && K > 0) ? (size_t)O * (size_t)((K + KC - 1) / KC * KC) : 0; }

extern "C" int svnet_binweight_pack_i8(const float* W, int64_t O, int64_t K, int8_t* w_i8, void* stream) {
    SVNET_REQUIRE(W && w_i8 && O > 0 && K > 0 && O * ((K + KC - 1) / KC * KC) < ((int64_t)1 << 31), SVNET_E_ARG, "svnet_binweight_pack_i8: bad arguments");
    const int Kp = (int)((K + KC - 1) / KC * KC);
    hipLaunchKernelGGL(binweight_pack_i8_kernel, dim3(svnet_grid(O * Kp, 256)), dim3(256), 0, (hipStream_t)stream, W, (int)O, (int)K, Kp, w_i8);
    SVNET_CHECK_LAUNCH("binweight_pack_i8_kernel");
    return SVNET_OK;
}

static int binlinear_i8_launch(const float* x, int64_t ldx, const float* beta, const int8_t* w_i8, const float* scale,
                               const float* bias, int64_t M, int64_t K, int64_t O, float* y, uint64_t* x_sign, uint64_t* x_nz,
                               uint64_t* x_ste, double* col_sums, const float* cloud_n, int64_t rows_per_cloud, void* stream) {
    SVNET_REQUIRE(x && beta && w_i8 && scale && y, SVNET_E_ARG, "svnet_binlinear_i8_fwd_f32: null pointer");
    SVNET_REQUIRE(!cloud_n || (rows_per_cloud > 0 && M % rows_per_cloud == 0), SVNET_E_ARG,
                  "svnet_binlinear_i8_cloud_fwd_f32: rows_per_cloud must divide M");
    SVNET_REQUIRE(M >= 0 && K > 0 && O > 0 && ldx >= K, SVNET_E_ARG, "svnet_binlinear_i8_fwd_f32: bad sizes");
    const bool any = x_sign || x_nz || x_ste, all = x_sign && x_nz && x_ste;
    SVNET_REQUIRE(!any || all, SVNET_E_ARG, "svnet_binlinear_i8_fwd_f32: pass all three saved planes or none");
    SVNET_REQUIRE(K < (1 << 24) && O < (1 << 24), SVNET_E_UNSUPPORTED, "svnet_binlinear_i8_fwd_f32: K=%lld, O=%lld too large", (long long)K, (long long)O);
    SVNET_REQUIRE(!col_sums || K <= 46340, SVNET_E_UNSUPPORTED, "svnet_binlinear_i8_fwd_f32: column sums need K <= 46340 (got %lld)", (long long)K);
    if (M == 0) return SVNET_OK;
    const int Kp = (int)((K + KC - 1) / KC * KC);
    const int ntw = O <= 128 ? 1 : (O <= 256 ? 2 : 4);
    const dim3 grid((unsigned)svnet_cdiv(M, BM), (unsigned)svnet_cdiv(O, 128 * ntw));
    const size_t lds = (size_t)BM * LDA + (size_t)128 * ntw * LDA + 3 * BM * 2 * sizeof(uint64_t);
    bool ok = true;
    if (ntw == 1) SVNET_LDS_OPTIN(ok, BM * LDA + 128 * LDA + 6144, "binlinear_i8_fwd_kernel<1>", reinterpret_cast<const void*>(&binlinear_i8_fwd_kernel<1>));
    else if (ntw == 2) SVNET_LDS_OPTIN(ok, BM * LDA + 256 * LDA + 6144, "binlinear_i8_fwd_kernel<2>", reinterpret_cast<const void*>(&binlinear_i8_fwd_kernel<2>));
    else SVNET_LDS_OPTIN(ok, BM * LDA + 512 * LDA + 6144, "binlinear_i8_fwd_kernel<4>", reinterpret_cast<const void*>(&binlinear_i8_fwd_kernel<4>));
    if (!ok) return SVNET_E_LAUNCH;
#define SVNET_BL_LAUNCH(NTW_)                                                                                                          \
    hipLaunchKernelGGL((binlinear_i8_fwd_kernel<NTW_>), grid, dim3(1024), lds, (hipStream_t)stream, x, ldx, beta, w_i8, scale, bias, M, (int)K, \
                       (int)O, Kp, y, reinterpret_cast<uint32_t*>(x_sign), reinterpret_cast<uint32_t*>(x_nz), reinterpret_cast<uint32_t*>(x_ste), col_sums, \
                       cloud_n, rows_per_cloud > 0 ? rows_per_cloud : 1)
    if (ntw == 1) SVNET_BL_LAUNCH(1);
    else if (ntw == 2) SVNET_BL_LAUNCH(2);
    else SVNET_BL_LAUNCH(4);
#undef SVNET_BL_LAUNCH
    SVNET_CHECK_LAUNCH("binlinear_i8_fwd_kernel");
    return SVNET_OK;
}

extern "C" int svnet_binlinear_i8_fwd_f32(const float* x, int64_t ldx, const float* beta, const int8_t* w_i8, const float* scale,
                                          const float* bias, int64_t M, int64_t K, int64_t O, float* y, uint64_t* x_sign, uint64_t* x_nz,
                                          uint64_t* x_ste, double* col_sums, void* stream) {
    return binlinear_i8_launch(x, ldx, beta, w_i8, scale, bias, M, K, O, y, x_sign, x_nz, x_ste, col_sums, nullptr, 0, stream);
}

extern "C" int svnet_binlinear_i8_cloud_fwd_f32(const float* x, int64_t ldx, const float* beta, const int8_t* w_i8, const float* scale,
                                                const float* bias, int64_t M, int64_t K, int64_t O, float* y, uint64_t* x_sign,
                                                uint64_t* x_nz, uint64_t* x_ste, double* col_sums, const float* cloud_n,
                                                int64_t rows_per_cloud, void* stream) {
    SVNET_REQUIRE(cloud_n, SVNET_E_ARG, "svnet_binlinear_i8_cloud_fwd_f32: null cloud counts");
    return binlinear_i8_launch(x, ldx, beta, w_i8, scale, bias, M, K, O, y, x_sign, x_nz, x_ste, col_sums, cloud_n, rows_per_cloud, stream);
}
```

svnet_amd/csrc/v2s.hip:

```cpp
#include "common.h"

namespace {

constexpr int J = 3;

template <int G>
__device__ __forceinline__ float group_sum(float v) { return group_sum_dpp<G>(v); }

constexpr int V2S_SUM_ROWS = 4, V2S_SUM_COLS = 8;
template <int G, int CPL, bool SUM = false>
__global__ __launch_bounds__(256) void v2s_fwd_kernel(const float* __restrict__ v, const float* __restrict__ w, int64_t M, int C,
                                                      float* __restrict__ s, int64_t s_ld, float* __restrict__ z_out,
                                                      const float* __restrict__ pre, int pre_cols, double* __restrict__ pre_sum = nullptr,
                                                      int64_t rows_per_cloud = 0) {
    constexpr int GPB = 256 / G;
    const int g = threadIdx.x % G;
    const int64_t group = SUM ? (int64_t)blockIdx.x * (GPB * V2S_SUM_ROWS) + threadIdx.x / G : ((int64_t)blockIdx.x * blockDim.x + threadIdx.x) / G;
    const int64_t ngroups = SUM ? GPB : ((int64_t)gridDim.x * blockDim.x) / G;
    float psum[SUM ? V2S_SUM_COLS : 1];
#pragma unroll
    for (int q = 0; q < (SUM ? V2S_SUM_COLS : 1); ++q) psum[q] = 0.f;
    float wr[J][CPL];
#pragma unroll
    for (int t = 0; t < CPL; ++t) {
        const int c = g + G * t;
#pragma unroll
        for (int j = 0; j < J; ++j) wr[j][t] = (c < C) ? w[j * C + c] : 0.f;
    }
    const int64_t iters = SUM ? V2S_SUM_ROWS : (M + ngroups - 1) / ngroups;
    for (int64_t it = 0; it < iters; ++it) {
        const int64_t m = group + it * ngroups;
        const bool live = m < M;
        float x[3][CPL];
#pragma unroll
        for (int i = 0; i < 3; ++i)
#pragma unroll
            for (int t = 0; t < CPL; ++t) {
                const int c = g + G * t;
                x[i][t] = (live && c < C) ? v[(m * 3 + i) * C + c] : 0.f;
            }
        float z[3][J];
#pragma unroll
        for (int i = 0; i < 3; ++i)
#pragma unroll
            for (int j = 0; j < J; ++j) {
                float p = 0.f;
#pragma unroll
                for (int t = 0; t < CPL; ++t) p = fmaf(x[i][t], wr[j][t], p);
                z[i][j] = group_sum<G>(p);
            }
        if (live) {
#pragma unroll
            for (int t = 0; t < CPL; ++t) {
                const int c = g + G * t;
                if (c < C) {
#pragma unroll
                    for (int j = 0; j < J; ++j)
                        s[m * s_ld + c * J + j] = x[0][t] * z[0][j] + x[1][t] * z[1][j] + x[2][t] * z[2][j];
                }
            }
            if (SUM) {
#pragma unroll
                for (int q = 0; q < V2S_SUM_COLS; ++q) {
                    const int c = g + G * q;
                    if (c < pre_cols) { const float t = pre[m * pre_cols + c]; s[m * s_ld - pre_cols + c] = t; psum[q] += t; }
                }
            } else if (pre) for (int c = g; c < pre_cols; c += G) s[m * s_ld - pre_cols + c] = pre[m * pre_cols + c];
            if (z_out && g == 0) {
#pragma unroll
                for (int i = 0; i < 3; ++i)
#pragma unroll
                    for (int j = 0; j < J; ++j) z_out[(m * 3 + i) * J + j] = z[i][j];
            }
        }
    }
    if constexpr (SUM) {
        __shared__ float part[GPB][G * V2S_SUM_COLS];
        const int gi = threadIdx.x / G;
#pragma unroll
        for (int q = 0; q < V2S_SUM_COLS; ++q) part[gi][g + G * q] = psum[q];
        __syncthreads();
        const int64_t cloud = ((int64_t)blockIdx.x * (GPB * V2S_SUM_ROWS)) / rows_per_cloud;
        for (int c = threadIdx.x; c < pre_cols; c += blockDim.x) {
            float t = 0.f;
#pragma unroll
            for (int q = 0; q < GPB; ++q) t += part[q][c];
            atomicAdd(&pre_sum[cloud * pre_cols + c], (double)t);
        }
    }
}

template <int G, int CPL>
__global__ __launch_bounds__(256) void v2s_bwd_kernel(const float* __restrict__ v, const float* __restrict__ w,
                                                      const float* __restrict__ ds, int64_t ds_ld, const float* __restrict__ dz_in, int64_t M,
                                                      int C, float* __restrict__ dv, float* __restrict__ GX) {
    __shared__ float gx_lds[J * 768];
    const int g = threadIdx.x % G;
    const int64_t group = ((int64_t)blockIdx.x * blockDim.x + threadIdx.x) / G;
    const int64_t ngroups = ((int64_t)gridDim.x * blockDim.x) / G;
    for (int e = threadIdx.x; e < J * C; e += blockDim.x) gx_lds[e] = 0.f;
    __syncthreads();
    float wr[J][CPL], gx[J][CPL];
#pragma unroll
    for (int t = 0; t < CPL; ++t) {
        const int c = g + G * t;
#pragma unroll
        for (int j = 0; j < J; ++j) {
            wr[j][t] = (c < C) ? w[j * C + c] : 0.f;
            gx[j][t] = 0.f;
        }
    }
    const int64_t iters = (M + ngroups - 1) / ngroups;
    for (int64_t it = 0; it < iters; ++it) {
        const int64_t m = group + it * ngroups;
        const bool live = m < M;
        float x[3][CPL], d[CPL][J];
#pragma unroll
        for (int t = 0; t < CPL; ++t) {
            const int c = g + G * t;
            const bool ok = live && c < C;
#pragma unroll
            for (int i = 0; i < 3; ++i) x[i][t] = ok ? v[(m * 3 + i) * C + c] : 0.f;
#pragma unroll
            for (int j = 0; j < J; ++j) d[t][j] = ok ? ds[m * ds_ld + c * J + j] : 0.f;
        }
        float z[3][J], dz[3][J];
#pragma unroll
        for (int i = 0; i < 3; ++i)
#pragma unroll
            for (int j = 0; j < J; ++j) {
                float pz = 0.f, pd = 0.f;
#pragma unroll
                for (int t = 0; t < CPL; ++t) {
                    pz = fmaf(x[i][t], wr[j][t], pz);
                    pd = fmaf(d[t][j], x[i][t], pd);
                }
                z[i][j] = group_sum<G>(pz);
                dz[i][j] = group_sum<G>(pd) + ((live && dz_in) ? dz_in[(m * 3 + i) * J + j] : 0.f);
            }
        if (live) {
#pragma unroll
            for (int t = 0; t < CPL; ++t) {
                const int c = g + G * t;
                if (c < C) {
#pragma unroll
                    for (int i = 0; i < 3; ++i) {
                        float a = 0.f;
#pragma unroll
                        for (int j = 0; j < J; ++j) a += d[t][j] * z[i][j] + dz[i][j] * wr[j][t];
                        dv[(m * 3 + i) * C + c] = a;
                    }
#pragma unroll
                    for (int j = 0; j < J; ++j) gx[j][t] += dz[0][j] * x[0][t] + dz[1][j] * x[1][t] + dz[2][j] * x[2][t];
                }
            }
        }
    }
#pragma unroll
    for (int t = 0; t < CPL; ++t) {
        const int c = g + G * t;
        if (c < C) {
#pragma unroll
            for (int j = 0; j < J; ++j) atomicAdd(&gx_lds[j * C + c], gx[j][t]);
        }
    }
    __syncthreads();
    float* gsl = svnet_slice_ptr(GX, J * C);
    for (int e = threadIdx.x; e < J * C; e += blockDim.x) atomicAdd(&gsl[e], gx_lds[e]);
}

template <int G, int CPL>
__global__ __launch_bounds__(256) void vproject_fwd_kernel(const float* __restrict__ v, const float* __restrict__ z, int64_t M, int C,
                                                           float* __restrict__ s) {
    const int g = threadIdx.x % G;
    const int64_t group = ((int64_t)blockIdx.x * blockDim.x + threadIdx.x) / G;
    const int64_t ngroups = ((int64_t)gridDim.x * blockDim.x) / G;
    for (int64_t m = group; m < M; m += ngroups) {
        float zz[3][J];
#pragma unroll
        for (int i = 0; i < 3; ++i)
#pragma unroll
            for (int j = 0; j < J; ++j) zz[i][j] = z[(m * 3 + i) * J + j];
#pragma unroll
        for (int t = 0; t < CPL; ++t) {
            const int c = g + G * t;
            if (c < C) {
                const float x0 = v[(m * 3 + 0) * C + c], x1 = v[(m * 3 + 1) * C + c], x2 = v[(m * 3 + 2) * C + c];
#pragma unroll
                for (int j = 0; j < J; ++j) s[m * C * J + c * J + j] = x0 * zz[0][j] + x1 * zz[1][j] + x2 * zz[2][j];
            }
        }
    }
}

template <int G, int CPL>
__global__ __launch_bounds__(256) void vproject_bwd_kernel(const float* __restrict__ v, const float* __restrict__ z,
                                                           const float* __restrict__ ds, int64_t M, int C, float* __restrict__ dv,
                                                           float* __restrict__ dz) {
    const int g = threadIdx.x % G;
    const int64_t group = ((int64_t)blockIdx.x * blockDim.x + threadIdx.x) / G;
    const int64_t ngroups = ((int64_t)gridDim.x * blockDim.x) / G;
    const int64_t iters = (M + ngroups - 1) / ngroups;
    for (int64_t it = 0; it < iters; ++it) {
        const int64_t m = group + it * ngroups;
        const bool live = m < M;
        float zz[3][J], pd[3][J];
#pragma unroll
        for (int i = 0; i < 3; ++i)
#pragma unroll
            for (int j = 0; j < J; ++j) {
                zz[i][j] = live ? z[(m * 3 + i) * J + j] : 0.f;
                pd[i][j] = 0.f;
            }
#pragma unroll
        for (int t = 0; t < CPL; ++t) {
            const int c = g + G * t;
            const bool ok = live && c < C;
            float x[3], d[J];
#pragma unroll
            for (int i = 0; i < 3; ++i) x[i] = ok ? v[(m * 3 + i) * C + c] : 0.f;
#pragma unroll
            for (int j = 0; j < J; ++j) d[j] = ok ? ds[m * C * J + c * J + j] : 0.f;
#pragma unroll
            for (int i = 0; i < 3; ++i) {
                float a = 0.f;
#pragma unroll
                for (int j = 0; j < J; ++j) {
                    a = fmaf(d[j], zz[i][j], a);
                    pd[i][j] = fmaf(d[j], x[i], pd[i][j]);
                }
                if (ok) dv[(m * 3 + i) * C + c] = a;
            }
        }
#pragma unroll
        for (int i = 0; i < 3; ++i)
#pragma unroll
            for (int j = 0; j < J; ++j) {
                const float tot = group_sum<G>(pd[i][j]);
                if (live && g == 0) dz[(m * 3 + i) * J + j] = tot;
            }
    }
}

inline unsigned v2s_grid(int64_t M, int G) {
    const int64_t groups_per_block = 256 / G;
    int64_t blocks = svnet_cdiv(M, groups_per_block * 4);
    if (blocks > 256 * 8) blocks = 256 * 8;
    if (blocks < 1) blocks = 1;
    return (unsigned)blocks;
}

}

static int v2s_fwd_launch(const float* v, const float* w_eff, int64_t M, int64_t C, int64_t Jn, float* s, int64_t s_ld, float* z_out,
                          const float* pre, int64_t pre_cols, void* stream, double* pre_sum = nullptr, int64_t rows_per_cloud = 0) {
    SVNET_REQUIRE(v && w_eff && s && M >= 0 && C > 0 && s_ld >= C * J + (pre ? pre_cols : 0) && (!pre || pre_cols > 0), SVNET_E_ARG,
                  "svnet_v2s_fwd_f32: bad arguments");
    SVNET_REQUIRE(Jn == J && C <= 768, SVNET_E_UNSUPPORTED, "svnet_v2s_fwd_f32: needs multi == 3 and C <= 768 (got %lld, %lld)",
                  (long long)Jn, (long long)C);
    if (M == 0) return SVNET_OK;
    hipStream_t st = (hipStream_t)stream;
#define SVNET_V2S(G, CPL) hipLaunchKernelGGL((v2s_fwd_kernel<G, CPL>), dim3(v2s_grid(M, G)), dim3(256), 0, st, v, w_eff, M, (int)C, s, s_ld, z_out, pre, (int)pre_cols)
    if (pre_sum) {
        const int G_ = C <= 96 ? 32 : 64;
        SVNET_REQUIRE(C > 24 && C <= 192 && pre && pre_cols <= (int64_t)V2S_SUM_COLS * G_ && rows_per_cloud > 0 && M % rows_per_cloud == 0 &&
                          rows_per_cloud % ((256 / G_) * V2S_SUM_ROWS) == 0, SVNET_E_UNSUPPORTED,
                      "svnet_v2s_cat_sum_fwd_f32: C=%lld, pre_cols=%lld, rows_per_cloud=%lld not supported", (long long)C, (long long)pre_cols,
                      (long long)rows_per_cloud);
        const unsigned blocks = (unsigned)(M / ((256 / G_) * V2S_SUM_ROWS));
        if (G_ == 32) hipLaunchKernelGGL((v2s_fwd_kernel<32, 3, true>), dim3(blocks), dim3(256), 0, st, v, w_eff, M, (int)C, s, s_ld, z_out, pre, (int)pre_cols, pre_sum, rows_per_cloud);
        else hipLaunchKernelGGL((v2s_fwd_kernel<64, 3, true>), dim3(blocks), dim3(256), 0, st, v, w_eff, M, (int)C, s, s_ld, z_out, pre, (int)pre_cols, pre_sum, rows_per_cloud);
        SVNET_CHECK_LAUNCH("v2s_fwd_kernel<sum>");
        return SVNET_OK;
    }
    if (C <= 3) SVNET_V2S(1, 3);
    else if (C <= 24) SVNET_V2S(8, 3);
    else if (C <= 96) SVNET_V2S(32, 3);
    else if (C <= 192) SVNET_V2S(64, 3);
    else if (C <= 384) SVNET_V2S(64, 6);
    else SVNET_V2S(64, 12);
#undef SVNET_V2S
    SVNET_CHECK_LAUNCH("v2s_fwd_kernel");
    return SVNET_OK;
}
extern "C" int svnet_v2s_fwd_f32(const float* v, const float* w_eff, int64_t M, int64_t C, int64_t Jn, float* s, float* z_out,
                                 void* stream) {
    return v2s_fwd_launch(v, w_eff, M, C, Jn, s, C * J, z_out, nullptr, 0, stream);
}
extern "C" int svnet_v2s_cat_fwd_f32(const float* v, const float* w_eff, const float* pre, int64_t pre_cols, int64_t M, int64_t C,
                                     int64_t Jn, float* out, int64_t out_ld, void* stream) {
    SVNET_REQUIRE(pre && out && pre_cols > 0, SVNET_E_ARG, "svnet_v2s_cat_fwd_f32: bad arguments");
    return v2s_fwd_launch(v, w_eff, M, C, Jn, out + pre_cols, out_ld, nullptr, pre, pre_cols, stream);
}

extern "C" int svnet_v2s_cat_sum_supported(int64_t M, int64_t C, int64_t pre_cols, int64_t rows_per_cloud) {
    const int64_t G_ = C <= 96 ? 32 : 64;
    return (C > 24 && C <= 192 && pre_cols > 0 && pre_cols <= (int64_t)V2S_SUM_COLS * G_ && rows_per_cloud > 0 && M > 0 && M % rows_per_cloud == 0 &&
            rows_per_cloud % ((256 / G_) * V2S_SUM_ROWS) == 0) ? 1 : 0;
}
extern "C" int svnet_v2s_cat_sum_fwd_f32(const float* v, const float* w_eff, const float* pre, int64_t pre_cols, int64_t M, int64_t C,
                                         int64_t Jn, float* out, int64_t out_ld, double* pre_sum, int64_t rows_per_cloud, void* stream) {
    SVNET_REQUIRE(pre && out && pre_cols > 0 && pre_sum, SVNET_E_ARG, "svnet_v2s_cat_sum_fwd_f32: bad arguments");
    return v2s_fwd_launch(v, w_eff, M, C, Jn, out + pre_cols, out_ld, nullptr, pre, pre_cols, stream, pre_sum, rows_per_cloud);
}

extern "C" int svnet_v2s_bwd_ld_f32(const float* v, const float* w_eff, const float* ds, int64_t ds_ld, const float* dz_in, int64_t M,
                                    int64_t C, int64_t Jn, float* dv, float* GX, void* stream);
extern "C" int svnet_v2s_bwd_f32(const float* v, const float* w_eff, const float* ds, const float* dz_in, int64_t M, int64_t C,
                                 int64_t Jn, float* dv, float* GX, void* stream) {
    return svnet_v2s_bwd_ld_f32(v, w_eff, ds, C * J, dz_in, M, C, Jn, dv, GX, stream);
}
extern "C" int svnet_v2s_bwd_ld_f32(const float* v, const float* w_eff, const float* ds, int64_t ds_ld, const float* dz_in, int64_t M,
                                    int64_t C, int64_t Jn, float* dv, float* GX, void* stream) {
    SVNET_REQUIRE(v && w_eff && ds && dv && GX && M >= 0 && C > 0 && ds_ld >= C * J, SVNET_E_ARG, "svnet_v2s_bwd_f32: bad arguments");
    SVNET_REQUIRE(Jn == J && C <= 768, SVNET_E_UNSUPPORTED, "svnet_v2s_bwd_f32: needs multi == 3 and C <= 768 (got %lld, %lld)",
                  (long long)Jn, (long long)C);
    if (M == 0) return SVNET_OK;
    hipStream_t st = (hipStream_t)stream;
#define SVNET_V2S(G, CPL) hipLaunchKernelGGL((v2s_bwd_kernel<G, CPL>), dim3(v2s_grid(M, G)), dim3(256), 0, st, v, w_eff, ds, ds_ld, dz_in, M, (int)C, dv, GX)
    if (C <= 3) SVNET_V2S(1, 3);
    else if (C <= 24) SVNET_V2S(8, 3);
    else if (C <= 96) SVNET_V2S(32, 3);
    else if (C <= 192) SVNET_V2S(64, 3);
    else if (C <= 384) SVNET_V2S(64, 6);
    else SVNET_V2S(64, 12);
#undef SVNET_V2S
    SVNET_CHECK_LAUNCH("v2s_bwd_kernel");
    return SVNET_OK;
}

extern "C" int svnet_vproject_fwd_f32(const float* v, const float* z, int64_t M, int64_t C, int64_t Jn, float* s, void* stream) {
    SVNET_REQUIRE(v && z && s && M >= 0 && C > 0, SVNET_E_ARG, "svnet_vproject_fwd_f32: bad arguments");
    SVNET_REQUIRE(Jn == J && C <= 768, SVNET_E_UNSUPPORTED, "svnet_vproject_fwd_f32: needs multi == 3 and C <= 768 (got %lld, %lld)",
                  (long long)Jn, (long long)C);
    if (M == 0) return SVNET_OK;
    hipStream_t st = (hipStream_t)stream;
#define SVNET_VP(G, CPL) hipLaunchKernelGGL((vproject_fwd_kernel<G, CPL>), dim3(v2s_grid(M, G)), dim3(256), 0, st, v, z, M, (int)C, s)
    if (C <= 24) SVNET_VP(8, 3);
    else if (C <= 96) SVNET_VP(32, 3);
    else if (C <= 192) SVNET_VP(64, 3);
    else if (C <= 384) SVNET_VP(64, 6);
    else SVNET_VP(64, 12);
#undef SVNET_VP
    SVNET_CHECK_LAUNCH("vproject_fwd_kernel");
    return SVNET_OK;
}

extern "C" int svnet_vproject_bwd_f32(const float* v, const float* z, const float* ds, int64_t M, int64_t C, int64_t Jn, float* dv,
                                      float* dz, void* stream) {
    SVNET_REQUIRE(v && z && ds && dv && dz && M >= 0 && C > 0, SVNET_E_ARG, "svnet_vproject_bwd_f32: bad arguments");
    SVNET_REQUIRE(Jn == J && C <= 768, SVNET_E_UNSUPPORTED, "svnet_vproject_bwd_f32: needs multi == 3 and C <= 768 (got %lld, %lld)",
                  (long long)Jn, (long long)C);
    if (M == 0) return SVNET_OK;
    hipStream_t st = (hipStream_t)stream;
#define SVNET_VP(G, CPL) hipLaunchKernelGGL((vproject_bwd_kernel<G, CPL>), dim3(v2s_grid(M, G)), dim3(256), 0, st, v, z, ds, M, (int)C, dv, dz)
    if (C <= 24) SVNET_VP(8, 3);
    else if (C <= 96) SVNET_VP(32, 3);
    else if (C <= 192) SVNET_VP(64, 3);
    else if (C <= 384) SVNET_VP(64, 6);
    else SVNET_VP(64, 12);
#undef SVNET_VP
    SVNET_CHECK_LAUNCH("vproject_bwd_kernel");
    return SVNET_OK;
}
```

svnet_amd/models/sv_layers.py:

```python
import os
import sys
import copy
import math
import numpy as np

import torch
import torch.nn as nn
import torch.nn.init as init
import torch.nn.functional as F

from .. import _ops
from .. import config
from .utils.sv_util import svpool, EdgeFeatures, XyzEdges

EPS = 1e-6

__all__ = ["EPS", "linear_bn_act", "Linear", "Conv1d", "VectorBN", "Vector2Scalar", "VectorReLU", "SVBlock", "SVFuse", "SV_STNkd",
           "svpool", "torch", "nn", "F", "np", "math", "os", "sys", "copy", "init"]

_ACT_NONE, _ACT_LEAKY, _ACT_RELU = 0, 1, 2


def _bn_momentum(bn):
    if bn.momentum is None:
        raise NotImplementedError("svnet_amd: BatchNorm1d(momentum=None) (cumulative average) is not supported")
    return float(bn.momentum)


def batch_norm_act(bn, x, act=_ACT_NONE, slope=0.2):
    training = bn.training or bn.running_mean is None
    nbt = bn.num_batches_tracked if (bn.training and bn.track_running_stats) else None
    return _ops.BNAct.apply(x, bn.weight, bn.bias, bn.running_mean, bn.running_var, training, act, slope, nbt, bn.eps, _bn_momentum(bn))


def linear_bn_act(lin, bn, x, act=_ACT_NONE, slope=0.2):
    if (config.FUSE_HEAD and isinstance(lin, Linear) and lin.bw and lin.ba and lin.bias is None and x.dim() == 2 and x.is_cuda
            and _ops.BinLinearBNAct.supported(x.shape[0], lin.in_features, lin.out_features) and bn.affine
            and lin.training == bn.training):
        training = bn.training or bn.running_mean is None
        grads = torch.is_grad_enabled() and (x.requires_grad or any(p.requires_grad for p in lin.parameters())
                                             or any(p.requires_grad for p in bn.parameters()))
        if training or not grads:
            nbt = bn.num_batches_tracked if (bn.training and bn.track_running_stats) else None
            return _ops.BinLinearBNAct.apply(x, lin.weight, lin.beta, lin.scale, bn.weight, bn.bias, bn.running_mean, bn.running_var,
                                             training, act, slope, nbt, bn.eps, _bn_momentum(bn), grads)
    return batch_norm_act(bn, lin(x), act, slope)


class Linear(nn.Linear):

    def __init__(self, in_channels, out_channels, bias, bw=False, ba=False):
        super(Linear, self).__init__(in_channels, out_channels, bias)
        self.bw, self.ba = bw, ba
        if ba:
            self.beta = nn.Parameter(torch.zeros(1, in_channels))
        if bw:
            self.scale = nn.Parameter(torch.ones(1, out_channels) / math.sqrt(in_channels))

    def forward(self, x, vstats=False):
        if self.bw and self.ba:
            return _ops.BinLinear.apply(x, self.weight, self.beta, self.scale, self.bias, self.training)
        if self.bw:
            y = _ops.BwLinear.apply(x, self.weight, self.scale, self.training, bool(vstats) and self.bias is None)
            return y if self.bias is None else y + self.bias
        if self.ba:
            raise AttributeError("'Linear' object has no attribute 'scale'")
        return _ops.FpLinear.apply(x, self.weight, self.bias)


class Conv1d(nn.Conv1d):

    def __init__(self, in_channels, out_channels, binary=False):
        super(Conv1d, self).__init__(in_channels, out_channels, 1, bias=False)
        print('Conv1d: ', in_channels, out_channels)
        self.binary = binary
        if binary:
            self.beta = nn.Parameter(torch.zeros(1, in_channels, 1))
            self.scale = nn.Parameter(torch.ones(1, out_channels, 1) / math.sqrt(in_channels))

    def forward_rows(self, rows):
        if self.binary:
            return _ops.BinLinear.apply(rows, self.weight, self.beta, self.scale, None, self.training)
        return _ops.FpLinear.apply(rows, self.weight.view(self.out_channels, self.in_channels), None)

    def forward(self, x):
        return self.forward_rows(x.transpose(1, 2)).transpose(1, 2).contiguous()


class VectorBN(nn.Module):

    def __init__(self, dim):
        super(VectorBN, self).__init__()
        self.bn = nn.BatchNorm1d(dim)

    def forward(self, v, gate=None):
        bn = self.bn
        training = bn.training or bn.running_mean is None
        nbt = bn.num_batches_tracked if bn.training else None
        rows = v.numel() // (3 * v.shape[-1])
        rows_per_batch = max(rows // v.shape[0], 1)
        return _ops.VBN.apply(v, bn.weight, bn.bias, bn.running_mean, bn.running_var, gate, rows_per_batch, training, nbt, bn.eps,
                              _bn_momentum(bn))


class Vector2Scalar(nn.Module):

    def __init__(self, v_dim, multi, binary=False, trans_back=False):
        super(Vector2Scalar, self).__init__()
        self.trans_back = trans_back
        self.linear = Linear(v_dim, multi, bias=False, bw=binary)

    def forward(self, v):
        assert v.ndim in [3, 4, 5], 'dim of v should be in [4, 5], got {}'.format(v.ndim)
        if isinstance(v, XyzEdges):
            if not self.linear.bw and not self.trans_back and tuple(self.linear.weight.shape) == (3, v.nc):
                return LazyInitScalar(self, v)
            v = v.materialize()
        s, z = _ops.V2S.apply(v, self.linear.weight, self.linear.scale if self.linear.bw else None, self.training)
        return (s, z) if self.trans_back else s


class VectorReLU(nn.Module):

    def __init__(self):
        super(VectorReLU, self).__init__()
        self.div = 10

    def forward(self, x):
        shape_x = x.shape
        rows = x.reshape(shape_x[0], -1, 3, shape_x[-1])
        kth = rows.shape[1] // self.div
        length = torch.linalg.vector_norm(rows, dim=2, keepdim=True).detach()
        threshold = torch.kthvalue(length, kth, dim=1, keepdim=True)[0]
        return torch.where(length > threshold, rows, torch.zeros_like(rows)).view(shape_x)


class LazyInitScalar:

    def __init__(self, v2s, edges):
        self.v2s, self.edges, self._s = v2s, edges, None

    def materialize(self):
        if self._s is None:
            self._s = self.v2s(self.edges.materialize())
        return self._s

    def __getattr__(self, name):
        return getattr(self.materialize(), name)


class PendingXyzBlock:

    def __init__(self, block, s_lazy, edges):
        self.block, self.s_lazy, self.edges, self._out = block, s_lazy, edges, None

    def pooled(self, dim, keepdim, spool):
        if dim != 2 or spool != 'max' or self._out is not None:
            return None
        b, e = self.block, self.edges
        bn1, bn2 = b.bn1, b.bn2.bn
        s, v, s_view, v_view = _ops.XyzBlock.apply(
            e.pts, e.idx, e.k, b.training, self.s_lazy.v2s.linear.weight, b.v2s.linear.weight, b.linear1.weight, bn1.weight,
            bn1.bias, bn1.running_mean, bn1.running_var, b.linear2.weight, bn2.weight, bn2.bias, bn2.running_mean, bn2.running_var,
            b.gate[0].weight, b.gate[2].weight, bn1.num_batches_tracked, bn2.num_batches_tracked)
        if s_view is not None:
            _ops._SINK.tracked(s_view, v_view)
        return (s.unsqueeze(2), v.unsqueeze(2)) if keepdim else (s, v)

    def materialize(self):
        if self._out is None:
            self._out = self.block._forward_rows((self.s_lazy.materialize(), self.edges.materialize()))
        return self._out

    def __iter__(self):
        return iter(self.materialize())

    def __getitem__(self, i):
        return self.materialize()[i]

    def __len__(self):
        return 2


class PendingEdgeBlock:

    def __init__(self, block, edges):
        self.block, self.edges, self._out = block, edges, None

    def pooled(self, dim, keepdim, spool):
        if dim != 2 or spool != 'max' or self._out is not None:
            return None
        b, e = self.block, self.edges
        bn1, bn2 = b.bn1, b.bn2.bn
        training = b.training
        if not training and torch.is_grad_enabled() and (e.s.requires_grad or any(p.requires_grad for p in b.parameters())):
            return None
        s, v, s_view, v_view = _ops.EdgeBlock.apply(
            e.s, e.v, e, e.k, training, b.v2s.linear.weight, b.v2s.linear.scale, b.linear1.weight, b.linear1.beta,
            b.linear1.scale, bn1.weight, bn1.bias, bn1.running_mean, bn1.running_var, b.linear2.weight, b.linear2.scale,
            bn2.weight, bn2.bias, bn2.running_mean, bn2.running_var, b.gate[0].weight, b.gate[2].weight,
            bn1.num_batches_tracked, bn2.num_batches_tracked)
        if s_view is not None:
            _ops._SINK.tracked(s_view, v_view)
        return (s.unsqueeze(2), v.unsqueeze(2)) if keepdim else (s, v)

    def materialize(self):
        if self._out is None:
            self._out = self.block._forward_rows(self.edges.materialize())
        return self._out

    def __iter__(self):
        return iter(self.materialize())

    def __getitem__(self, i):
        return self.materialize()[i]

    def __len__(self):
        return 2


class SVBlock(nn.Module):

    def __init__(self, in_dims, out_dims, binary=False):
        super(SVBlock, self).__init__()
        print('SVBlock: ', in_dims, out_dims)

        self.gate = nn.Sequential(
            nn.Linear(in_dims[0], out_dims[1] // 2, bias=False),
            nn.ReLU(inplace=True),
            nn.Linear(out_dims[1] // 2, out_dims[1], bias=False),
            nn.Sigmoid(),
        )
        self.v2s = Vector2Scalar(in_dims[1], 3, binary=binary)

        self.linear1 = Linear(in_dims[0] + in_dims[1] * 3, out_dims[0], bias=False, bw=binary, ba=binary)
        self.bn1 = nn.BatchNorm1d(out_dims[0])
        self.relu = nn.LeakyReLU(negative_slope=0.2)

        self.linear2 = Linear(in_dims[1], out_dims[1], bias=False, bw=binary)
        self.bn2 = VectorBN(out_dims[1])

    def _gate(self, s):
        small = self.gate[0].out_features <= 256 and self.gate[2].out_features <= 256
        s3 = s.reshape(s.shape[0], -1, s.shape[-1])
        if small and config.GATE_MEAN_INSIDE and _ops.GateMLPRows.supported(s3):
            return _ops.GateMLPRows.apply(s3, self.gate[0].weight, self.gate[2].weight)
        pooled = _ops.Pool.apply(s3, 1, 1)
        if small:
            return _ops.GateMLP.apply(pooled, self.gate[0].weight, self.gate[2].weight)
        h = _ops.Act.apply(_ops.FpLinear.apply(pooled, self.gate[0].weight, None), 1)
        _ops._tap_act(self.gate[0].weight, 2, h)
        return _ops.Act.apply(_ops.FpLinear.apply(h, self.gate[2].weight, None), 2)

    def _can_fuse(self, edges):
        lin1, lin2 = self.linear1, self.linear2
        if not (lin1.bw and lin1.ba and lin2.bw and self.v2s.linear.bw) or edges.idx_is_global:
            return False
        Cs, Cv = edges.s.shape[-1], edges.v.shape[-1]
        return (Cs <= 64 and 2 * Cv <= 64 and lin1.out_features <= 128 and lin2.out_features <= 64 and 2 <= edges.k <= 64
                and edges.s.shape[1] <= 8192 and lin1.out_features in (8, 16, 32, 64, 128) and lin1.in_features == 2 * Cs + 6 * Cv
                and self._default_bn())

    def _default_bn(self):
        return all(bn.track_running_stats and bn.eps == _ops.BN_EPS and bn.momentum == _ops.BN_MOMENTUM for bn in (self.bn1, self.bn2.bn))

    def forward(self, x):
        if isinstance(x, EdgeFeatures) and self._can_fuse(x):
            return PendingEdgeBlock(self, x)
        if isinstance(x, (tuple, list)) and len(x) == 2 and (isinstance(x[0], LazyInitScalar) or isinstance(x[1], XyzEdges)):
            s, v = x
            lin1, lin2 = self.linear1, self.linear2
            if (isinstance(s, LazyInitScalar) and s.edges is v and not (lin1.bw or lin1.ba or lin2.bw or self.v2s.linear.bw)
                    and lin1.in_features == 6 * v.nc and lin2.in_features == v.nc and lin1.out_features <= 64 and lin2.out_features <= 64
                    and v.k <= 64 and self._default_bn()
                    and (self.training or not torch.is_grad_enabled()
                         or not any(p.requires_grad for p in self.parameters()))):
                return PendingXyzBlock(self, s, v)
            x = (s.materialize() if isinstance(s, LazyInitScalar) else s, v.materialize() if isinstance(v, XyzEdges) else v)
        return self._forward_rows(x)

    def _v2s_cat_fusable(self, s, v):
        lin = self.v2s.linear
        return (config.FUSE_V2S_CAT and torch.is_tensor(s) and torch.is_tensor(v) and s.is_cuda and not self.v2s.trans_back
                and lin.weight.shape[0] == 3 and v.shape[-1] <= 768 and s.shape[:-1] == v.shape[:-2])

    def _cat_s_v2s(self, s, v):
        lin = self.v2s.linear
        if self._v2s_cat_fusable(s, v):
            return _ops.V2SCat.apply(s, v, lin.weight, lin.scale if lin.bw else None, self.training)
        return torch.cat([s, self.v2s(v)], dim=-1)

    def _cat_and_gate(self, s, v):
        lin = self.v2s.linear
        if not (self._v2s_cat_fusable(s, v) and s.dim() >= 3 and s.shape[-1] >= 128 and self.gate[0].out_features <= 256
                and self.gate[2].out_features <= 256):
            return None
        if config.FUSE_CAT_MEAN:
            return _ops.V2SCat.apply(s, v, lin.weight, lin.scale if lin.bw else None, self.training, s.shape[0], self.gate[0].weight,
                                     self.gate[2].weight)
        cat, s_mean = _ops.V2SCat.apply(s, v, lin.weight, lin.scale if lin.bw else None, self.training, s.shape[0])
        return cat, _ops.GateMLP.apply(s_mean, self.gate[0].weight, self.gate[2].weight)

    def forward_prebn(self, x):
        return self._forward_rows(x, prebn=True)

    def forward_pretail(self, x):
        return self._forward_rows(x, prebn=True, pretail=True)

    def forward_cloud_s(self, s_point, s_cloud, v):
        lin1 = self.linear1
        B, N, Cp = s_point.shape
        Cc = s_cloud.shape[-1]
        binary = lin1.bw and lin1.ba
        ok = (config.SPLIT_BROADCAST and (binary or not (lin1.bw or lin1.ba)) and lin1.bias is None and s_point.is_cuda
              and self._v2s_cat_fusable(s_point, v) and lin1.in_features == Cp + Cc + 3 * v.shape[-1] and B * N >= 1024
              and lin1.out_features >= 64 and self.gate[0].out_features <= 256 and self.gate[2].out_features <= 256)
        if not ok:
            return self.forward((torch.cat([s_point, s_cloud.unsqueeze(1).expand(B, N, Cc)], dim=-1), v))
        lz = self.v2s.linear
        two = config.TWO_STREAM_BLOCKS and B * N >= config.TWO_STREAM_MIN_ROWS
        if two:
            main, side = torch.cuda.current_stream(s_point.device), _ops._side_stream(s_point.device)
            side.wait_stream(main)
            with torch.cuda.stream(side):
                v_lin = self.linear2(v, vstats=True)
        cat_pt, mean_pt = _ops.V2SCat.apply(s_point, v, lz.weight, lz.scale if lz.bw else None, self.training, B)
        v_scale = _ops.GateMLP.apply(torch.cat([mean_pt, s_cloud], dim=-1), self.gate[0].weight, self.gate[2].weight)
        if binary:
            y = _ops.BinLinearCloud.apply(s_cloud, cat_pt, lin1.weight, lin1.beta, lin1.scale, self.training, Cp)
        else:
            W = lin1.weight
            y = _ops.FpLinear.apply(cat_pt, torch.cat([W[:, :Cp], W[:, Cp + Cc:]], dim=1), None) \
                + _ops.FpLinear.apply(s_cloud, W[:, Cp:Cp + Cc], None).unsqueeze(1)
        s_out = batch_norm_act(self.bn1, y, _ACT_LEAKY, self.relu.negative_slope)
        if two:
            side.wait_stream(main)
            with torch.cuda.stream(side):
                v_out = self.bn2(v_lin, gate=v_scale)
            main.wait_stream(side)
            v_out.record_stream(main)
        else:
            v_out = self.bn2(self.linear2(v, vstats=True), gate=v_scale)
        return (s_out, v_out)

    def _forward_rows(self, x, prebn=False, pretail=False):
        s, v = x
        rows = s.numel() // max(s.shape[-1], 1)
        if config.TWO_STREAM_BLOCKS and rows >= config.TWO_STREAM_MIN_ROWS and s.is_cuda:
            main, side = torch.cuda.current_stream(s.device), _ops._side_stream(s.device)
            side.wait_stream(main)
            with torch.cuda.stream(side):
                v_lin = self.linear2(v, vstats=True)
            fused = self._cat_and_gate(s, v)
            if fused is not None:
                s_cat, v_scale = fused
            else:
                v_scale = self._gate(s)
            if pretail:
                return (self.linear1(s_cat if fused is not None else self._cat_s_v2s(s, v)), v_lin, v_scale)
            side.wait_stream(main)
            with torch.cuda.stream(side):
                v_out = self.bn2(v_lin, gate=v_scale)
            s_out = self.linear1(s_cat if fused is not None else self._cat_s_v2s(s, v))
            if not prebn:
                s_out = batch_norm_act(self.bn1, s_out, _ACT_LEAKY, self.relu.negative_slope)
            main.wait_stream(side)
            v_out.record_stream(main)
            return (s_out, v_out)

        v_scale = self._gate(s)
        s = self.linear1(self._cat_s_v2s(s, v))
        if not prebn:
            s = batch_norm_act(self.bn1, s, _ACT_LEAKY, self.relu.negative_slope)

        v = self.linear2(v, vstats=True)
        if pretail:
            return (s, v, v_scale)
        v = self.bn2(v, gate=v_scale)
        return (s, v)


class SVFuse(nn.Module):

    def __init__(self, v_dim, multi, binary, trans_back=False):
        super(SVFuse, self).__init__()
        print('SVFuse: ', v_dim)
        self.trans_back = trans_back
        self.v2s = Vector2Scalar(v_dim, multi, binary=binary, trans_back=trans_back)

    def parts(self, x):
        s, v = x
        return s, self.v2s(v)

    def forward(self, x):
        s, v = x
        if self.trans_back:
            s_v, trans = self.v2s(v)
            return torch.cat([s, s_v], dim=-1), trans
        lin = self.v2s.linear
        if (config.FUSE_V2S_CAT and torch.is_tensor(s) and torch.is_tensor(v) and s.is_cuda and lin.weight.shape[0] == 3 and v.shape[-1] <= 768
                and s.shape[:-1] == v.shape[:-2] and s.dim() >= 2):
            return _ops.V2SCat.apply(s, v, lin.weight, lin.scale if lin.bw else None, self.training)
        return torch.cat([s, self.v2s(v)], dim=-1)


class SV_STNkd(nn.Module):

    def __init__(self, dim, binary):
        super(SV_STNkd, self).__init__()
        widths = [dim, (64 // 2, 64 // 6), (128 // 2, 128 // 6), (1024 // 2, 1024 // 6),
                  (512 // 2, 512 // 6), (256 // 2, 256 // 6), dim]
        names = ['conv1', 'conv2', 'conv3', 'fc1', 'fc2', 'fc3']
        for i, name in enumerate(names):
            setattr(self, name, SVBlock(widths[i], widths[i + 1], binary=binary))

    def forward(self, x):
        for name in ('conv1', 'conv2', 'conv3'):
            x = getattr(self, name)(x)
        x = svpool(x, dim=1)
        for name in ('fc1', 'fc2', 'fc3'):
            x = getattr(self, name)(x)
        return x
```

Measured before the change: 7752 point-clouds/sec.

## Fuse V2S concat with ternary int8 activation packing before binlinear MFMA

Adds a V2S-concat kernel that quantizes the concatenated features straight into ternary int8 rows laid out for the MFMA GEMM. It also writes the sign, nonzero and STE bit planes and the per-cloud sums for the gate. The binlinear int8 kernel gains a template path that reads these pre-packed int8 activations instead of float x plus beta. The goal is to avoid materializing the f32 concat tensor and re-quantizing it inside the GEMM. The new path applies only to the pretail case under several shape conditions, and it reuses the existing backward functions through a shim context.

```diff
diff --git a/include/svnet_hip.h b/include/svnet_hip.h
--- a/include/svnet_hip.h
+++ b/include/svnet_hip.h
@@ -91,6 +91,8 @@
 int svnet_binlinear_i8_fwd_f32(const float* x, int64_t ldx, const float* beta, const int8_t* w_i8, const float* scale,
                                const float* bias, int64_t M, int64_t K, int64_t O, float* y, uint64_t* x_sign, uint64_t* x_nz,
                                uint64_t* x_ste, double* col_sums, void* stream);
+int svnet_binlinear_i8_op_fwd_f32(const int8_t* a8, const int8_t* w_i8, const float* scale, const float* bias, int64_t M, int64_t K,
+                                  int64_t O, float* y, double* col_sums, void* stream);
 int svnet_binlinear_i8_cloud_fwd_f32(const float* x, int64_t ldx, const float* beta, const int8_t* w_i8, const float* scale,
                                      const float* bias, int64_t M, int64_t K, int64_t O, float* y, uint64_t* x_sign, uint64_t* x_nz,
                                      uint64_t* x_ste, double* col_sums, const float* cloud_n, int64_t rows_per_cloud, void* stream);
@@ -242,6 +244,10 @@
 int svnet_v2s_cat_sum_supported(int64_t M, int64_t C, int64_t pre_cols, int64_t rows_per_cloud);
 int svnet_v2s_cat_sum_fwd_f32(const float* v, const float* w_eff, const float* pre, int64_t pre_cols, int64_t M, int64_t C, int64_t multi,
                               float* out, int64_t out_ld, double* pre_sum, int64_t rows_per_cloud, void* stream);
+int svnet_v2s_cat_i8_supported(int64_t M, int64_t C, int64_t pre_cols, int64_t rows_per_cloud);
+int svnet_v2s_cat_i8_fwd_f32(const float* v, const float* w_eff, const float* pre, int64_t pre_cols, int64_t M, int64_t C, int64_t multi,
+                             const float* beta, int8_t* a8, uint64_t* x_sign, uint64_t* x_nz, uint64_t* x_ste, double* pre_sum,
+                             int64_t rows_per_cloud, void* stream);
 int svnet_v2s_bwd_ld_f32(const float* v, const float* w_eff, const float* ds, int64_t ds_ld, const float* dz_in, int64_t M, int64_t C,
                          int64_t J, float* dv, float* GX, void* stream);
 int svnet_vproject_fwd_f32(const float* v, const float* z, int64_t M, int64_t C, int64_t J, float* s, void* stream);
diff --git a/svnet_amd/_lib.py b/svnet_amd/_lib.py
--- a/svnet_amd/_lib.py
+++ b/svnet_amd/_lib.py
@@ -178,11 +178,14 @@
     "svnet_binweight_i8_bytes": (c_sz, [c_i64, c_i64]),
     "svnet_binweight_pack_i8": (c_int, [c_p, c_i64, c_i64, c_p, c_p]),
     "svnet_binlinear_i8_fwd_f32": (c_int, [c_p, c_i64, c_p, c_p, c_p, c_p, c_i64, c_i64, c_i64, c_p, c_p, c_p, c_p, c_p, c_p]),
+    "svnet_binlinear_i8_op_fwd_f32": (c_int, [c_p, c_p, c_p, c_p, c_i64, c_i64, c_i64, c_p, c_p, c_p]),
     "svnet_binlinear_i8_cloud_fwd_f32": (c_int, [c_p, c_i64, c_p, c_p, c_p, c_p, c_i64, c_i64, c_i64, c_p, c_p, c_p, c_p, c_p, c_p, c_i64, c_p]),
     "svnet_v2s_fwd_f32": (c_int, [c_p, c_p, c_i64, c_i64, c_i64, c_p, c_p, c_p]),
     "svnet_v2s_bwd_f32": (c_int, [c_p, c_p, c_p, c_p, c_i64, c_i64, c_i64, c_p, c_p, c_p]),
     "svnet_v2s_cat_fwd_f32": (c_int, [c_p, c_p, c_p, c_i64, c_i64, c_i64, c_i64, c_p, c_i64, c_p]),
     "svnet_v2s_cat_sum_supported": (c_int, [c_i64, c_i64, c_i64, c_i64]),
+    "svnet_v2s_cat_i8_supported": (c_int, [c_i64, c_i64, c_i64, c_i64]),
+    "svnet_v2s_cat_i8_fwd_f32": (c_int, [c_p, c_p, c_p, c_i64, c_i64, c_i64, c_i64, c_p, c_p, c_p, c_p, c_p, c_p, c_i64, c_p]),
     "svnet_v2s_cat_sum_fwd_f32": (c_int, [c_p, c_p, c_p, c_i64, c_i64, c_i64, c_i64, c_p, c_i64, c_p, c_i64, c_p]),
     "svnet_v2s_bwd_ld_f32": (c_int, [c_p, c_p, c_p, c_i64, c_p, c_i64, c_i64, c_i64, c_p, c_p, c_p]),
     "svnet_vproject_fwd_f32": (c_int, [c_p, c_p, c_i64, c_i64, c_i64, c_p, c_p]),
diff --git a/svnet_amd/_ops.py b/svnet_amd/_ops.py
--- a/svnet_amd/_ops.py
+++ b/svnet_amd/_ops.py
@@ -969,6 +969,89 @@
             call("svnet_slices_sum_f32", _p(gxb), J * C, _stream())
             dW, dsc = gxb[:J * C].view(J, C), None
         return ds, dv.view(vshape), dW, dsc, None, None, dW0, dW2
+
+
+class _PartCtx:
+
+    def __init__(self, saved, needs_input_grad, **attrs):
+        self.saved_tensors, self.needs_input_grad = saved, needs_input_grad
+        self.__dict__.update(attrs)
+
+
+class V2SCatBinLinear(torch.autograd.Function):
+
+    @staticmethod
+    def supported(M, C, Cs, clouds, O):
+        return (clouds > 0 and M % clouds == 0 and M >= 1024 and O >= 64
+                and bool(_lib.lib().svnet_v2s_cat_i8_supported(M, C, Cs, M // clouds)))
+
+    @staticmethod
+    def forward(ctx, s, v, Wz, scz, gate_W0, gate_W2, W1, beta1, scale1, training=True):
+        global _FUSED_COLSUMS
+        _hip(s, v, Wz, scz, gate_W0, gate_W2, W1, beta1, scale1)
+        training = bool(training)
+        v3 = _f32c(v).reshape(-1, 3, v.shape[-1])
+        M, _, C = v3.shape
+        s2 = _f32c(s).reshape(M, s.shape[-1])
+        Cs, clouds = s2.shape[1], s.shape[0]
+        rows = M // clouds
+        dev = v.device
+        Wzc, sczc = _f32c(Wz), _f32c(scz).view(-1)
+        J = Wzc.shape[0]
+        w_eff = _binweight(Wz, scz)["w_eff"]
+        W1_in, W1c = W1, _f32c(W1).reshape(W1.shape[0], -1)
+        O, K = W1c.shape
+        sc1, bt1 = _f32c(scale1).view(-1), _f32c(beta1).view(-1)
+        need_grad = any(ctx.needs_input_grad)
+        packed = _binweight(W1_in, scale1, i8=True)
+        planes = ([torch.empty(((M + 63) // 64, K), dtype=torch.int64, device=dev) for _ in range(3)] if (need_grad or TAP is not None)
+                  else [None] * 3)
+        s_sum = _zeros((clouds, Cs), torch.float64, dev)
+        a8 = torch.empty((M, (K + 127) // 128 * 128), dtype=torch.int8, device=dev)
+        call("svnet_v2s_cat_i8_fwd_f32", _p(v3), _p(w_eff), _p(s2), Cs, M, C, J, _p(bt1), _p(a8), _p(planes[0]), _p(planes[1]), _p(planes[2]),
+             _p(s_sum), rows, _stream())
+        W0c, W2c = _f32c(gate_W0), _f32c(gate_W2)
+        H, Ov = W0c.shape[0], W2c.shape[0]
+        pooled = torch.empty((clouds, Cs), dtype=torch.float32, device=dev)
+        h = torch.empty((clouds, H), dtype=torch.float32, device=dev)
+        gate = torch.empty((clouds, Ov), dtype=torch.float32, device=dev)
+        call("svnet_gate_mlp_fwd_f32", None, _p(s_sum), _p(pooled), 1.0 / float(rows), _p(W0c), _p(W2c), clouds, Cs, H, Ov, _p(h), _p(gate),
+             None, 0, _stream())
+        _tap_act(gate_W0, 2, h)
+        sums = _zeros((_sliced_len(2 * O),), torch.float64, dev) if (training and config.FUSE_BN_STATS and K <= 46340) else None
+        y = torch.empty((M, O), dtype=torch.float32, device=dev)
+        call("svnet_binlinear_i8_op_fwd_f32", _p(a8), _p(packed["w_i8"]), _p(sc1), None, M, K, O, _p(y), _p(sums), _stream())
+        _FUSED_COLSUMS = (y, y._version, sums) if sums is not None else None
+        if TAP is not None:
+            TAP["signs"].append(("rows", M, K, planes))
+        if need_grad:
+            ctx.save_for_backward(v3, Wzc, w_eff, sczc, pooled, W0c, W2c, h, gate, W1c, sc1, packed["w_b"], *planes)
+        cat_shape = s.shape[:-1] + (K,)
+        ctx.training = training
+        ctx.v2s_meta = (M, C, J, Cs, s.shape, v.shape, scz.shape)
+        ctx.lin_meta = (M, K, O, _words(K), cat_shape, beta1.shape, scale1.shape, False, W1_in.shape)
+        ctx.clouds, ctx.gate_in_scale = clouds, 1.0 / float(rows)
+        ctx.defer_ok = defer_rows_wgrad.on
+        ctx.set_materialize_grads(False)
+        return y.view(s.shape[:-1] + (O,)), gate
+
+    @staticmethod
+    def backward(ctx, gy, ggate):
+        saved = ctx.saved_tensors
+        nig = ctx.needs_input_grad
+        M, K, O = ctx.lin_meta[:3]
+        if gy is None:
+            gy = torch.zeros((M, O), dtype=torch.float32, device=saved[0].device)
+        cat_grad = any(nig[:6])
+        lin = _PartCtx(saved[9:], (cat_grad, nig[6], nig[7], nig[8], False, False), training=ctx.training, meta=ctx.lin_meta,
+                       defer_ok=ctx.defer_ok)
+        dcat, dW1, dbeta1, dsc1, _, _ = BinLinear.backward(lin, gy)
+        ds = dv = dWz = dscz = dW0 = dW2 = None
+        if cat_grad and dcat is not None:
+            cat = _PartCtx(saved[:9], nig[:4] + (False, False) + nig[4:6], training=ctx.training, meta=ctx.v2s_meta, clouds=ctx.clouds,
+                           with_gate=True, gate_in_scale=ctx.gate_in_scale)
+            ds, dv, dWz, dscz, _, _, dW0, dW2 = V2SCat.backward(cat, dcat, ggate)
+        return ds, dv, dWz, dscz, dW0, dW2, dW1, dbeta1, dsc1, None
 
 
 class VProject(torch.autograd.Function):
diff --git a/svnet_amd/config.py b/svnet_amd/config.py
--- a/svnet_amd/config.py
+++ b/svnet_amd/config.py
@@ -41,3 +41,4 @@
 KNN_TABLE_AHEAD = True
 FUSE_BLOCK_TAIL = True
 FUSE_CAT_MEAN = True
+V2S_CAT_I8 = True
diff --git a/svnet_amd/csrc/binlinear_mfma.hip b/svnet_amd/csrc/binlinear_mfma.hip
--- a/svnet_amd/csrc/binlinear_mfma.hip
+++ b/svnet_amd/csrc/binlinear_mfma.hip
@@ -20,8 +20,8 @@
     }
 }
 
-template <int NTW>
-__global__ __launch_bounds__(1024, 4) void binlinear_i8_fwd_kernel(const float* __restrict__ x, int64_t ldx, const float* __restrict__ beta,
+template <int NTW, bool I8IN = false>
+__global__ __launch_bounds__(1024, 4) void binlinear_i8_fwd_kernel(const float* __restrict__ x, const int8_t* __restrict__ a8, int64_t ldx, const float* __restrict__ beta,
                                                                    const int8_t* __restrict__ w8, const float* __restrict__ scale,
                                                                    const float* __restrict__ bias, int64_t M, int K, int O, int Kp,
                                                                    float* __restrict__ y, uint32_t* __restrict__ x_sign32,
@@ -39,7 +39,7 @@
     const int wr = wave >> 2, wc = wave & 3;
     const int64_t m0 = (int64_t)blockIdx.x * BM;
     const int o0 = blockIdx.y * OT;
-    const bool save = x_sign32 != nullptr && blockIdx.y == 0;
+    const bool save = !I8IN && x_sign32 != nullptr && blockIdx.y == 0;
 
     i32x16 acc[NTW];
 #pragma unroll
@@ -50,7 +50,7 @@
     const int nchunks = Kp / KC;
     float xa[4][4];
     const int64_t brow = min(m0 + 8 * wave, M - 1);
-    const float* xbase = x + brow * ldx;
+    const float* xbase = I8IN ? nullptr : x + brow * ldx;
     uint32_t rowb[4];
 #pragma unroll
     for (int rp = 0; rp < 4; ++rp) rowb[rp] = (uint32_t)(min(m0 + 8 * wave + h + 2 * rp, M - 1) - brow) * (uint32_t)ldx * 4u;
@@ -61,7 +61,10 @@
         _Pragma("unroll") for (int rp = 0; rp < 4; ++rp)                                          \
             _Pragma("unroll") for (int j = 0; j < 4; ++j) xa[rp][j] = ld_f32_sbase(xbase, rowb[rp] + colb_[j]); \
     } while (0)
-    SVNET_BL_LOAD_A(0);
+    const int8_t* arow = I8IN ? a8 + min(m0 + (tid >> 3), M - 1) * (int64_t)Kp + 16 * (tid & 7) : nullptr;
+    uint4 xa8;
+    if constexpr (I8IN) xa8 = *reinterpret_cast<const uint4*>(arow);
+    else SVNET_BL_LOAD_A(0);
     for (int c = 0; c < nchunks; ++c) {
         const int k0 = c * KC;
         uint4 bstage[NTW];
@@ -72,7 +75,9 @@
             const int o = min(o0 + n, O - 1);
             bstage[u] = *reinterpret_cast<const uint4*>(w8 + (int64_t)o * Kp + k0 + 16 * pc);
         }
-        {
+        if constexpr (I8IN) {
+            *reinterpret_cast<uint4*>(&At[(tid >> 3) * LDA + 16 * (tid & 7)]) = xa8;
+        } else {
             float bt[4];
 #pragma unroll
             for (int j = 0; j < 4; ++j) bt[j] = beta[min(k0 + 32 * j + r, K - 1)];
@@ -117,7 +122,8 @@
             *reinterpret_cast<uint4*>(&Bt[(e >> 3) * LDA + 16 * (e & 7)]) = bstage[u];
         }
         __syncthreads();
-        SVNET_BL_LOAD_A(min(k0 + KC, (nchunks - 1) * KC));
+        if constexpr (I8IN) xa8 = *reinterpret_cast<const uint4*>(arow + min(k0 + KC, (nchunks - 1) * KC));
+        else SVNET_BL_LOAD_A(min(k0 + KC, (nchunks - 1) * KC));
         __builtin_amdgcn_sched_barrier(0);
         if (save) {
             for (int item = wave; item < 24; item += 16) {
@@ -211,13 +217,13 @@
     return SVNET_OK;
 }
 
-static int binlinear_i8_launch(const float* x, int64_t ldx, const float* beta, const int8_t* w_i8, const float* scale,
+static int binlinear_i8_launch(const float* x, const int8_t* a8, int64_t ldx, const float* beta, const int8_t* w_i8, const float* scale,
                                const float* bias, int64_t M, int64_t K, int64_t O, float* y, uint64_t* x_sign, uint64_t* x_nz,
                                uint64_t* x_ste, double* col_sums, const float* cloud_n, int64_t rows_per_cloud, void* stream) {
-    SVNET_REQUIRE(x && beta && w_i8 && scale && y, SVNET_E_ARG, "svnet_binlinear_i8_fwd_f32: null pointer");
+    SVNET_REQUIRE((a8 ? !x && !beta && !x_sign && !cloud_n : x && beta) && w_i8 && scale && y, SVNET_E_ARG, "svnet_binlinear_i8_fwd_f32: null pointer");
     SVNET_REQUIRE(!cloud_n || (rows_per_cloud > 0 && M % rows_per_cloud == 0), SVNET_E_ARG,
                   "svnet_binlinear_i8_cloud_fwd_f32: rows_per_cloud must divide M");
-    SVNET_REQUIRE(M >= 0 && K > 0 && O > 0 && ldx >= K, SVNET_E_ARG, "svnet_binlinear_i8_fwd_f32: bad sizes");
+    SVNET_REQUIRE(M >= 0 && K > 0 && O > 0 && (a8 || ldx >= K), SVNET_E_ARG, "svnet_binlinear_i8_fwd_f32: bad sizes");
     const bool any = x_sign || x_nz || x_ste, all = x_sign && x_nz && x_ste;
     SVNET_REQUIRE(!any || all, SVNET_E_ARG, "svnet_binlinear_i8_fwd_f32: pass all three saved planes or none");
     SVNET_REQUIRE(K < (1 << 24) && O < (1 << 24), SVNET_E_UNSUPPORTED, "svnet_binlinear_i8_fwd_f32: K=%lld, O=%lld too large", (long long)K, (long long)O);
@@ -228,17 +234,25 @@
     const dim3 grid((unsigned)svnet_cdiv(M, BM), (unsigned)svnet_cdiv(O, 128 * ntw));
     const size_t lds = (size_t)BM * LDA + (size_t)128 * ntw * LDA + 3 * BM * 2 * sizeof(uint64_t);
     bool ok = true;
-    if (ntw == 1) SVNET_LDS_OPTIN(ok, BM * LDA + 128 * LDA + 6144, "binlinear_i8_fwd_kernel<1>", reinterpret_cast<const void*>(&binlinear_i8_fwd_kernel<1>));
-    else if (ntw == 2) SVNET_LDS_OPTIN(ok, BM * LDA + 256 * LDA + 6144, "binlinear_i8_fwd_kernel<2>", reinterpret_cast<const void*>(&binlinear_i8_fwd_kernel<2>));
-    else SVNET_LDS_OPTIN(ok, BM * LDA + 512 * LDA + 6144, "binlinear_i8_fwd_kernel<4>", reinterpret_cast<const void*>(&binlinear_i8_fwd_kernel<4>));
+#define SVNET_BL_KERNEL(NTW_, I8_) reinterpret_cast<const void*>(&binlinear_i8_fwd_kernel<NTW_, I8_>)
+    if (ntw == 1) SVNET_LDS_OPTIN(ok, BM * LDA + 128 * LDA + 6144, "binlinear_i8_fwd_kernel<1>", SVNET_BL_KERNEL(1, false), SVNET_BL_KERNEL(1, true));
+    else if (ntw == 2) SVNET_LDS_OPTIN(ok, BM * LDA + 256 * LDA + 6144, "binlinear_i8_fwd_kernel<2>", SVNET_BL_KERNEL(2, false), SVNET_BL_KERNEL(2, true));
+    else SVNET_LDS_OPTIN(ok, BM * LDA + 512 * LDA + 6144, "binlinear_i8_fwd_kernel<4>", SVNET_BL_KERNEL(4, false), SVNET_BL_KERNEL(4, true));
+#undef SVNET_BL_KERNEL
     if (!ok) return SVNET_E_LAUNCH;
-#define SVNET_BL_LAUNCH(NTW_)                                                                                                          \
-    hipLaunchKernelGGL((binlinear_i8_fwd_kernel<NTW_>), grid, dim3(1024), lds, (hipStream_t)stream, x, ldx, beta, w_i8, scale, bias, M, (int)K, \
-                       (int)O, Kp, y, reinterpret_cast<uint32_t*>(x_sign), reinterpret_cast<uint32_t*>(x_nz), reinterpret_cast<uint32_t*>(x_ste), col_sums, \
-                       cloud_n, rows_per_cloud > 0 ? rows_per_cloud : 1)
-    if (ntw == 1) SVNET_BL_LAUNCH(1);
-    else if (ntw == 2) SVNET_BL_LAUNCH(2);
-    else SVNET_BL_LAUNCH(4);
+#define SVNET_BL_LAUNCH(NTW_, I8_)                                                                                                     \
+    hipLaunchKernelGGL((binlinear_i8_fwd_kernel<NTW_, I8_>), grid, dim3(1024), lds, (hipStream_t)stream, x, a8, ldx, beta, w_i8, scale, bias, M, \
+                       (int)K, (int)O, Kp, y, reinterpret_cast<uint32_t*>(x_sign), reinterpret_cast<uint32_t*>(x_nz), reinterpret_cast<uint32_t*>(x_ste), \
+                       col_sums, cloud_n, rows_per_cloud > 0 ? rows_per_cloud : 1)
+    if (a8) {
+        if (ntw == 1) SVNET_BL_LAUNCH(1, true);
+        else if (ntw == 2) SVNET_BL_LAUNCH(2, true);
+        else SVNET_BL_LAUNCH(4, true);
+    } else {
+        if (ntw == 1) SVNET_BL_LAUNCH(1, false);
+        else if (ntw == 2) SVNET_BL_LAUNCH(2, false);
+        else SVNET_BL_LAUNCH(4, false);
+    }
 #undef SVNET_BL_LAUNCH
     SVNET_CHECK_LAUNCH("binlinear_i8_fwd_kernel");
     return SVNET_OK;
@@ -247,7 +261,13 @@
 extern "C" int svnet_binlinear_i8_fwd_f32(const float* x, int64_t ldx, const float* beta, const int8_t* w_i8, const float* scale,
                                           const float* bias, int64_t M, int64_t K, int64_t O, float* y, uint64_t* x_sign, uint64_t* x_nz,
                                           uint64_t* x_ste, double* col_sums, void* stream) {
-    return binlinear_i8_launch(x, ldx, beta, w_i8, scale, bias, M, K, O, y, x_sign, x_nz, x_ste, col_sums, nullptr, 0, stream);
+    return binlinear_i8_launch(x, nullptr, ldx, beta, w_i8, scale, bias, M, K, O, y, x_sign, x_nz, x_ste, col_sums, nullptr, 0, stream);
+}
+
+extern "C" int svnet_binlinear_i8_op_fwd_f32(const int8_t* a8, const int8_t* w_i8, const float* scale, const float* bias, int64_t M, int64_t K,
+                                             int64_t O, float* y, double* col_sums, void* stream) {
+    SVNET_REQUIRE(a8, SVNET_E_ARG, "svnet_binlinear_i8_op_fwd_f32: null operand");
+    return binlinear_i8_launch(nullptr, a8, 0, nullptr, w_i8, scale, bias, M, K, O, y, nullptr, nullptr, nullptr, col_sums, nullptr, 0, stream);
 }
 
 extern "C" int svnet_binlinear_i8_cloud_fwd_f32(const float* x, int64_t ldx, const float* beta, const int8_t* w_i8, const float* scale,
@@ -255,5 +275,5 @@
                                                 uint64_t* x_nz, uint64_t* x_ste, double* col_sums, const float* cloud_n,
                                                 int64_t rows_per_cloud, void* stream) {
     SVNET_REQUIRE(cloud_n, SVNET_E_ARG, "svnet_binlinear_i8_cloud_fwd_f32: null cloud counts");
-    return binlinear_i8_launch(x, ldx, beta, w_i8, scale, bias, M, K, O, y, x_sign, x_nz, x_ste, col_sums, cloud_n, rows_per_cloud, stream);
-}
+    return binlinear_i8_launch(x, nullptr, ldx, beta, w_i8, scale, bias, M, K, O, y, x_sign, x_nz, x_ste, col_sums, cloud_n, rows_per_cloud, stream);
+}
diff --git a/svnet_amd/csrc/v2s.hip b/svnet_amd/csrc/v2s.hip
--- a/svnet_amd/csrc/v2s.hip
+++ b/svnet_amd/csrc/v2s.hip
@@ -86,6 +86,116 @@
 #pragma unroll
             for (int q = 0; q < GPB; ++q) t += part[q][c];
             atomicAdd(&pre_sum[cloud * pre_cols + c], (double)t);
+        }
+    }
+}
+
+constexpr int V2S_I8_ROWS = 32, V2S_I8_KP_MAX = 1024;
+template <int G>
+__global__ __launch_bounds__(256) void v2s_cat_i8_kernel(const float* __restrict__ v, const float* __restrict__ w, int64_t M, int C,
+                                                         const float* __restrict__ pre, int pre_cols, const float* __restrict__ beta, int Kp,
+                                                         int8_t* __restrict__ a8, uint32_t* __restrict__ x_sign32, uint32_t* __restrict__ x_nz32,
+                                                         uint32_t* __restrict__ x_ste32, double* __restrict__ pre_sum, int64_t rows_per_cloud) {
+    constexpr int GPB = 256 / G, ITERS = V2S_I8_ROWS / GPB;
+    __shared__ __attribute__((aligned(16))) uint8_t code[V2S_I8_ROWS][V2S_I8_KP_MAX];
+    __shared__ float part[GPB][G * V2S_SUM_COLS];
+    const int K = pre_cols + C * J;
+    const int g = threadIdx.x % G, gi = threadIdx.x / G;
+    const int64_t m0 = (int64_t)blockIdx.x * V2S_I8_ROWS;
+    auto enc = [](float tv) -> uint8_t { return (uint8_t)((tv > 0.f) | ((tv < 0.f) << 1) | ((fabsf(tv) <= 1.2f) << 2)); };
+    float psum[V2S_SUM_COLS];
+#pragma unroll
+    for (int q = 0; q < V2S_SUM_COLS; ++q) psum[q] = 0.f;
+    float wr[J][3];
+#pragma unroll
+    for (int t = 0; t < 3; ++t) {
+        const int c = g + G * t;
+#pragma unroll
+        for (int j = 0; j < J; ++j) wr[j][t] = (c < C) ? w[j * C + c] : 0.f;
+    }
+    for (int it = 0; it < ITERS; ++it) {
+        const int rl = gi + GPB * it;
+        const int64_t m = m0 + rl;
+        float x[3][3];
+#pragma unroll
+        for (int i = 0; i < 3; ++i)
+#pragma unroll
+            for (int t = 0; t < 3; ++t) {
+                const int c = g + G * t;
+                x[i][t] = (c < C) ? v[(m * 3 + i) * C + c] : 0.f;
+            }
+        float z[3][J];
+#pragma unroll
+        for (int i = 0; i < 3; ++i)
+#pragma unroll
+            for (int j = 0; j < J; ++j) {
+                float p = 0.f;
+#pragma unroll
+                for (int t = 0; t < 3; ++t) p = fmaf(x[i][t], wr[j][t], p);
+                z[i][j] = group_sum<G>(p);
+            }
+#pragma unroll
+        for (int t = 0; t < 3; ++t) {
+            const int c = g + G * t;
+            if (c < C) {
+#pragma unroll
+                for (int j = 0; j < J; ++j) {
+                    const float sv = x[0][t] * z[0][j] + x[1][t] * z[1][j] + x[2][t] * z[2][j];
+                    code[rl][pre_cols + c * J + j] = enc(sv + beta[pre_cols + c * J + j]);
+                }
+            }
+        }
+#pragma unroll
+        for (int q = 0; q < V2S_SUM_COLS; ++q) {
+            const int c = g + G * q;
+            if (c < pre_cols) { const float t = pre[m * pre_cols + c]; code[rl][c] = enc(t + beta[c]); psum[q] += t; }
+        }
+    }
+    for (int e = threadIdx.x; e < V2S_I8_ROWS * (Kp - K); e += blockDim.x) code[e / (Kp - K)][K + e % (Kp - K)] = 0;
+#pragma unroll
+    for (int q = 0; q < V2S_SUM_COLS; ++q) part[gi][g + G * q] = psum[q];
+    __syncthreads();
+    const int64_t cloud = m0 / rows_per_cloud;
+    for (int c = threadIdx.x; c < pre_cols; c += blockDim.x) {
+        float t = 0.f;
+#pragma unroll
+        for (int q = 0; q < GPB; ++q) t += part[q][c];
+        atomicAdd(&pre_sum[cloud * pre_cols + c], (double)t);
+    }
+    const int nq = Kp / 16;
+    for (int e = threadIdx.x; e < V2S_I8_ROWS * nq; e += blockDim.x) {
+        const int r = e / nq, p = e - r * nq;
+        const int cb = 128 * (p >> 3) + 4 * (p & 7);
+        uint32_t in[4], out[4];
+#pragma unroll
+        for (int j = 0; j < 4; ++j) {
+            const uint32_t d = *reinterpret_cast<const uint32_t*>(&code[r][cb + 32 * j]);
+            in[j] = (d & 0x01010101u) | (((d >> 1) & 0x01010101u) * 0xFFu);
+        }
+#pragma unroll
+        for (int qq = 0; qq < 4; ++qq)
+            out[qq] = ((in[0] >> (8 * qq)) & 0xFFu) | (((in[1] >> (8 * qq)) & 0xFFu) << 8) | (((in[2] >> (8 * qq)) & 0xFFu) << 16) |
+                      (((in[3] >> (8 * qq)) & 0xFFu) << 24);
+        *reinterpret_cast<uint4*>(a8 + (m0 + r) * Kp + 16 * p) = make_uint4(out[0], out[1], out[2], out[3]);
+    }
+    if (x_sign32) {
+        const int64_t blk = m0 >> 6;
+        const int half = (int)((m0 >> 5) & 1);
+        const bool last_lo = half == 0 && m0 + V2S_I8_ROWS >= M;
+        for (int k = threadIdx.x; k < K; k += blockDim.x) {
+            uint32_t sg = 0, nz = 0, st = 0;
+#pragma unroll 8
+            for (int r = 0; r < V2S_I8_ROWS; ++r) {
+                const uint32_t b = code[r][k];
+                sg |= (b & 1u) << r;
+                nz |= ((b | (b >> 1)) & 1u) << r;
+                st |= ((b >> 2) & 1u) << r;
+            }
+            const int64_t at = (blk * K + k) * 2 + half;
+            x_sign32[at] = sg;
+            x_nz32[at] = nz;
+            x_ste32[at] = st;
+            if (last_lo) { x_sign32[at + 1] = 0u; x_nz32[at + 1] = 0u; x_ste32[at + 1] = 0u; }
         }
     }
 }
@@ -304,6 +414,28 @@
     return v2s_fwd_launch(v, w_eff, M, C, Jn, out + pre_cols, out_ld, nullptr, pre, pre_cols, stream, pre_sum, rows_per_cloud);
 }
 
+extern "C" int svnet_v2s_cat_i8_supported(int64_t M, int64_t C, int64_t pre_cols, int64_t rows_per_cloud) {
+    const int64_t K = pre_cols + C * J, Kp = (K + 127) / 128 * 128;
+    return (C > 24 && C <= 96 && pre_cols > 0 && pre_cols <= (int64_t)V2S_SUM_COLS * 32 && Kp <= V2S_I8_KP_MAX && rows_per_cloud > 0 && M > 0 &&
+            M % rows_per_cloud == 0 && rows_per_cloud % V2S_I8_ROWS == 0) ? 1 : 0;
+}
+extern "C" int svnet_v2s_cat_i8_fwd_f32(const float* v, const float* w_eff, const float* pre, int64_t pre_cols, int64_t M, int64_t C,
+                                        int64_t Jn, const float* beta, int8_t* a8, uint64_t* x_sign, uint64_t* x_nz, uint64_t* x_ste,
+                                        double* pre_sum, int64_t rows_per_cloud, void* stream) {
+    SVNET_REQUIRE(v && w_eff && pre && beta && a8 && pre_sum, SVNET_E_ARG, "svnet_v2s_cat_i8_fwd_f32: bad arguments");
+    const bool any = x_sign || x_nz || x_ste, all = x_sign && x_nz && x_ste;
+    SVNET_REQUIRE(!any || all, SVNET_E_ARG, "svnet_v2s_cat_i8_fwd_f32: pass all three planes or none");
+    SVNET_REQUIRE(Jn == J && svnet_v2s_cat_i8_supported(M, C, pre_cols, rows_per_cloud), SVNET_E_UNSUPPORTED,
+                  "svnet_v2s_cat_i8_fwd_f32: M=%lld, C=%lld, pre_cols=%lld, rows_per_cloud=%lld not supported", (long long)M, (long long)C,
+                  (long long)pre_cols, (long long)rows_per_cloud);
+    const int K = (int)(pre_cols + C * J), Kp = (K + 127) / 128 * 128;
+    hipLaunchKernelGGL((v2s_cat_i8_kernel<32>), dim3((unsigned)(M / V2S_I8_ROWS)), dim3(256), 0, (hipStream_t)stream, v, w_eff, M, (int)C,
+                       pre, (int)pre_cols, beta, Kp, a8, reinterpret_cast<uint32_t*>(x_sign), reinterpret_cast<uint32_t*>(x_nz),
+                       reinterpret_cast<uint32_t*>(x_ste), pre_sum, rows_per_cloud);
+    SVNET_CHECK_LAUNCH("v2s_cat_i8_kernel");
+    return SVNET_OK;
+}
+
 extern "C" int svnet_v2s_bwd_ld_f32(const float* v, const float* w_eff, const float* ds, int64_t ds_ld, const float* dz_in, int64_t M,
                                     int64_t C, int64_t Jn, float* dv, float* GX, void* stream);
 extern "C" int svnet_v2s_bwd_f32(const float* v, const float* w_eff, const float* ds, const float* dz_in, int64_t M, int64_t C,
diff --git a/svnet_amd/models/sv_layers.py b/svnet_amd/models/sv_layers.py
--- a/svnet_amd/models/sv_layers.py
+++ b/svnet_amd/models/sv_layers.py
@@ -300,6 +300,18 @@
                                      self.gate[2].weight)
         cat, s_mean = _ops.V2SCat.apply(s, v, lin.weight, lin.scale if lin.bw else None, self.training, s.shape[0])
         return cat, _ops.GateMLP.apply(s_mean, self.gate[0].weight, self.gate[2].weight)
+
+    def _cat_gate_linear1(self, s, v):
+        lin1, lz = self.linear1, self.v2s.linear
+        if not (config.V2S_CAT_I8 and config.FUSE_CAT_MEAN and config.BINLINEAR_MFMA and lin1.bw and lin1.ba and lin1.bias is None
+                and lz.bw and self._v2s_cat_fusable(s, v) and s.dim() == 3 and s.shape[-1] >= 128 and self.gate[0].out_features <= 256
+                and self.gate[2].out_features <= 256 and lin1.in_features == s.shape[-1] + 3 * v.shape[-1]):
+            return None
+        B, N, Cs = s.shape
+        if not _ops.V2SCatBinLinear.supported(B * N, v.shape[-1], Cs, B, lin1.out_features):
+            return None
+        return _ops.V2SCatBinLinear.apply(s, v, lz.weight, lz.scale, self.gate[0].weight, self.gate[2].weight, lin1.weight, lin1.beta,
+                                          lin1.scale, self.training)
 
     def forward_prebn(self, x):
         return self._forward_rows(x, prebn=True)
@@ -351,6 +363,10 @@
             side.wait_stream(main)
             with torch.cuda.stream(side):
                 v_lin = self.linear2(v, vstats=True)
+            if pretail:
+                fused_y = self._cat_gate_linear1(s, v)
+                if fused_y is not None:
+                    return (fused_y[0], v_lin, fused_y[1])
             fused = self._cat_and_gate(s, v)
             if fused is not None:
                 s_cat, v_scale = fused
```

Result: no change. 7820 point-clouds/sec, median of 6 (+0.9%).
